# noegroup/bgflow

Hardware: AMD Instinct MI355X
Metric: flow samples/s (fwd+log|detJ|) at batch 2^20 (higher is better)
Workload: dtype f32 (split-f16 conditioner GEMMs: hi+lo f16 operand pairs, f32 accumulate)

## Files before the change

bgflow_amd/_lib.py:

```python
import ctypes
import os

import torch

_HERE = os.path.dirname(os.path.abspath(__file__))
LIB_PATH = os.environ.get("BGK_LIB") or os.path.join(_HERE, "libbgflow_amd.so")
_lib = None

i32, i64, f32, f64, vp = ctypes.c_int32, ctypes.c_int64, ctypes.c_float, ctypes.c_double, ctypes.c_void_p

_SIGNATURES = {
    "bgk_abi_version": (ctypes.c_int, []),
    "bgk_last_error": (ctypes.c_char_p, []),
    "bgk_set_option": (ctypes.c_int, [i32, i32]),
    "bgk_detmath_probe": (ctypes.c_int, [vp, i64, i32, vp, vp]),
    "bgk_rqs_transform": (ctypes.c_int, [vp, i64, vp, i64, i32, vp, i64, i32, i32, i32,
                                         f64, f64, f64, f64, f64, f64, f64, i32,
                                         vp, i64, vp, i32, vp, vp, vp]),
    "bgk_rqs_backward": (ctypes.c_int, [vp, i64, vp, i64, i32, vp, i64, i32, i32, i32,
                                        f64, f64, f64, f64, f64, f64, f64, i32,
                                        vp, i64, vp, vp, i64, vp, i64, vp, i32, vp]),
    "bgk_affine_transform": (ctypes.c_int, [vp, i64, vp, i64, vp, i64, vp, i32, i32, i32, i64, i32,
                                            vp, i64, vp, i32, vp]),
    "bgk_affine_backward": (ctypes.c_int, [vp, i64, vp, i64, vp, i64, vp, i32, i32, i32, i64, i32,
# ... 18 lines not shown
                                     vp, vp, vp, i64, vp, i64, vp, i32, vp, vp]),
    "bgk_ic_ic2xyz": (ctypes.c_int, [vp, vp, vp, i64, vp, i64, vp, i32, vp, i32, i32, f32, i32,
                                     vp, vp, i32, f32, i64, vp, i64, vp, i32, vp, vp]),
    "bgk_ic_refsys": (ctypes.c_int, [vp, i64, i32, i32, f32, i32, vp, vp, i32, vp]),
    "bgk_icdf_ic2xyz": (ctypes.c_int, [vp, vp, vp, i64, vp, i64, vp, vp, vp, vp, i32, f32, vp, i32, vp, i32, i32, f32, i32,
                                       vp, vp, i32, f32, i64, vp, i64, vp, i32, vp, vp]),
    "bgk_icdf_ic2xyz_reg": (ctypes.c_int, [vp, vp, vp, vp, vp, i32, f32, vp, i32, vp, i32, f32, i32, vp, vp, i32, f64, i64,
                                           vp, i64, vp, i32, vp, vp]),
    "bgk_icdf_ic2xyz_uni": (ctypes.c_int, [vp, vp, vp, vp, vp, i32, f32, vp, i32, vp, i32, f32, i32, vp, vp, i32, f64, i64,
                                           vp, i64, vp, i32, vp, vp]),
    "bgk_icdf_ic2xyz_uni_train": (ctypes.c_int, [vp, vp, vp, vp, vp, i32, f32, vp, i32, vp, i32, f32, i32, vp, vp, i32, f64, i64,
                                                 vp, i64, vp, i32, vp, vp, vp, vp, vp, vp]),
    "bgk_icdf_ic2xyz_uni_train_kl": (ctypes.c_int, [vp, vp, vp, vp, vp, i32, f32, vp, i32, vp, i32, f32, i32, vp, vp, i32, f64, i64,
                                                    vp, i64, vp, vp, vp, vp, vp, vp, vp, f64, f64, f64, i32, vp, vp, vp, vp, vp]),
    "bgk_xyz2ic_cdf_uni": (ctypes.c_int, [vp, vp, i32, f32, vp, i32, vp, i32, f32, i32, vp, vp, i32, f64, i64,
                                          vp, vp, vp, vp, vp, i32, vp, vp]),
    "bgk_ic_ic2xyz_backward": (ctypes.c_int, [vp, vp, vp, i64, vp, i64, vp, i32, vp, i32, i32, f32, i32, vp, i32, i64,
                                              vp, i64, vp, vp, vp, vp, i64, vp, i64, vp, vp]),
    "bgk_cdf_transform": (ctypes.c_int, [vp, i64, vp, i64, i32, i32, i32, f32, vp, i64, vp, i32, vp]),
    "bgk_cdf_backward": (ctypes.c_int, [vp, i64, vp, i64, vp, i64, i32, i32, i32, f32, vp, i64, vp, vp, i64, vp]),
    "bgk_ic_xyz2ic_backward": (ctypes.c_int, [vp, i64, vp, i32, vp, i32, i32, f32, i32, vp, i32, i64,
                                              vp, vp, vp, i64, vp, i64, vp, vp, i64, vp]),
    "bgk_ic_refsys_backward": (ctypes.c_int, [vp, vp, vp, i64, i32, i32, f32, i32, vp, vp]),
    "bgk_coupling_rqs_dense": (ctypes.c_int, [vp, i64, i32, i32, vp, vp, vp, i32, i32, i32,
                                              vp, i64, i64, i32, i32, ctypes.c_uint64, i32,
                                              f64, f64, f64, f64, f64, f64, f64, i32,
                                              vp, i64, vp, i32, vp, vp, vp]),
    "bgk_coupling_rqs_dense_h2": (ctypes.c_int, [vp, i64, i32, i32, vp, vp, vp, f32, f32, f32, vp, i32, i32, i32, i32,
                                                 vp, i64, i64, i32, i32, ctypes.c_uint64, i32,
                                                 f64, f64, f64, f64, f64, f64, f64, i32,
                                                 vp, i64, vp, i32, vp, vp, vp]),
    "bgk_coupling_rqs_dense_deep": (ctypes.c_int, [vp, i64, i32, i32, vp, vp, vp, f32, vp, f32, i32, i32,
                                                   vp, i64, i64, i32, i32, ctypes.c_uint64, i32,
                                                   f64, f64, f64, f64, f64, f64, f64, i32,
                                                   vp, i64, vp, i32, vp, vp, vp]),
    "bgk_coupling_rqs_dense_h2_mc": (ctypes.c_int, [vp, vp, vp, i32, i32, vp, vp, vp, f32, f32, f32, vp, i32, i32, i32, i32,
                                                    vp, i64, i64, i32, i32, ctypes.c_uint64, i32,
                                                    f64, f64, f64, f64, f64, f64, f64, i32,
                                                    vp, i64, vp, i32, vp, vp, vp]),
    "bgk_coupling_affine_dense_h2_mc": (ctypes.c_int, [vp, vp, vp, i32, i32,
                                                       vp, vp, vp, f32, f32, f32, i32, vp, vp, vp, f32, f32, f32, i32,
                                                       i32, vp, i32, i32, i32, vp, i64, i64, i32, vp, i64, vp, i32, vp]),
    "bgk_coupling_affine_dense_h3_mc": (ctypes.c_int, [vp, vp, vp, i32, i32,
                                                       vp, vp, vp, vp, f32, f32, f32, f32, i32, vp, vp, vp, vp, f32, f32, f32, f32, i32,
                                                       i32, vp, i32, i32, i32, vp, i64, i64, i32, vp, i64, vp, i32, vp]),
    "bgk_pack_dense_h2": (ctypes.c_int, [vp, vp, i32, i32, vp, vp, vp, vp, i32, vp, i32, i32, i32, vp, vp, vp, vp, vp]),
    "bgk_coupling_rqs_dense_h2_train": (ctypes.c_int, [vp, i64, i32, i32, vp, vp, vp, f32, f32, f32, vp, i32, i32, i32,
                                                       vp, i64, i64, i32, i32, ctypes.c_uint64, i32,
                                                       f64, f64, f64, f64, f64, f64, f64, i32,
                                                       vp, i64, vp, i32, vp, vp, vp, vp, i64, vp, i32, vp]),
    "bgk_coupling_rqs_dense_h2_backward": (ctypes.c_int, [vp, vp, f32, vp, i32, i32, vp, i64, i64, i32, i32, i32, ctypes.c_uint64, i32,
                                                          f64, f64, f64, f64, f64, f64, f64, i32,
                                                          vp, i64, vp, vp, i64, vp, i64, vp, vp]),
    "bgk_coupling_affine_dense_h2": (ctypes.c_int, [vp, i64, i32, i32,
                                                    vp, vp, vp, f32, f32, f32, i32, vp, vp, vp, f32, f32, f32, i32,
                                                    i32, vp, i32, i32, i32, vp, i64, i64, i32, vp, i64, vp, i32, vp]),
    "bgk_coupling_affine_dense_h3": (ctypes.c_int, [vp, i64, i32, i32,
                                                    vp, vp, vp, vp, f32, f32, f32, f32, i32, vp, vp, vp, vp, f32, f32, f32, f32, i32,
                                                    i32, vp, i32, i32, i32, vp, i64, i64, i32, vp, i64, vp, i32, vp]),
    "bgk_coupling_affine_dense_deep": (ctypes.c_int, [vp, i64, i32, i32,
                                                      vp, vp, vp, f32, vp, f32, i32, vp, vp, vp, f32, vp, f32, i32,
                                                      i32, i32, vp, i32, i32, i32, vp, i64, i64, i32, vp, i64, vp, i32, vp]),
    "bgk_pack_dense_h2_t": (ctypes.c_int, [vp, i32, vp, vp, i32, vp, vp, vp, vp, vp]),
    "bgk_dense_backward_dx": (ctypes.c_int, [vp, i64, i32, vp, vp, vp, i64, i32, i32, vp, vp, vp, vp, i32, i64,
                                             vp, vp, vp, vp, vp, i64, vp, i64, vp, vp, vp]),
    "bgk_dense_weight_grad_reduce_many": (ctypes.c_int, [i32] + [vp] * 10 + [i32, vp]),
    "bgk_pack_dense_h2_many": (ctypes.c_int, [i32] + [vp] * 14 + [vp]),
    "bgk_pack_dense_h2_t_many": (ctypes.c_int, [i32] + [vp] * 9 + [vp]),
    "bgk_column_sum": (ctypes.c_int, [vp, i64, i64, i32, vp, i32, vp, vp]),
    "bgk_absmax": (ctypes.c_int, [vp, i64, i64, i32, vp, vp]),
    "bgk_whiten": (ctypes.c_int, [vp, i64, vp, vp, vp, i32, i32, i64, vp, i64, vp]),
    "bgk_normal_energy": (ctypes.c_int, [vp, i64, vp, i32, i64, f64, f64, vp, vp]),
    "bgk_normal_energy_backward": (ctypes.c_int, [vp, i64, vp, i32, i64, f64, vp, vp, i64, vp]),
    "bgk_energy_fields": (ctypes.c_int, [vp, vp, vp, vp, vp, vp, i32, i64, f64, f64, f64, vp, vp, i32, vp, i32, vp, vp]),
    "bgk_energy_fields_backward": (ctypes.c_int, [vp, vp, vp, vp, vp, vp, i32, i64, f64, vp, vp, vp, vp, i32, vp, vp, vp, vp]),
    "bgk_philox_fields": (ctypes.c_int, [ctypes.c_uint64, ctypes.c_uint32, i64, i32, vp, vp, vp, vp, vp, vp, vp, vp, f64, i64, vp, vp]),
    "bgk_colmap": (ctypes.c_int, [vp, i32, vp, i32, vp, vp, ctypes.c_uint64, ctypes.c_uint32, i64, i64, vp, i32, f64, vp, vp]),
    "bgk_grad_nan_flag":(ctypes.c_int, [vp, i64, vp, vp]),
    "bgk_adam_step": (ctypes.c_int, [vp, vp, vp, vp, i64, f32, f32, f32, f32, f32, i64, vp, vp, vp]),
    "bgk_dense_weight_grad_workspace": (i64, [i64, i32, i32]),
    "bgk_dense_weight_grad": (ctypes.c_int, [vp, i64, i32, vp, vp, vp, vp, i32, vp, i64, i32, i32, i64, vp, i64,
                                             vp, vp, vp, vp, vp, vp, i32, vp, vp]),
    "bgk_pack_rqs_columns": (i32, [i32, i32, vp, vp]),
    "bgk_dense_layer": (ctypes.c_int, [vp, i64, i64, i32, vp, i32, f32, vp, vp, i32, i32, vp, i64, i32, vp]),
    "bgk_pack_linear_layer": (ctypes.c_int, [vp, i64, i32, i32, vp, vp, vp]),
    "bgk_dense_layer_steps": (ctypes.c_int, [i32]),
    "bgk_refresh_linear_layer": (ctypes.c_int, [vp, i64, i32, i32, i32, vp, vp, vp, vp]),
    "bgk_activation": (ctypes.c_int, [vp, i64, i64, i32, i32, vp, i64, vp]),
    "bgk_activation_backward": (ctypes.c_int, [vp, i64, vp, i64, i64, i32, i32, vp, i64, vp]),
    "bgk_affine_net_backward64_workspace": (i64, [i64, i32, i32, i32, i32]),
    "bgk_affine_net_backward64": (ctypes.c_int, [vp, i64, i32, vp, vp, vp, i64, i32, i32, i32, vp, vp, vp, vp, i32, i64,
                                                 vp, i64, vp, i64, vp, vp, i64, vp, vp, vp, vp, vp, vp, i32, vp]),
    "bgk_affine_coupling_backward64_workspace": (i64, [i64, i32, i32, i32, i32, i32, i32]),
    "bgk_affine_coupling_backward64": (ctypes.c_int, [vp, i64, i32, vp, i64, i32, vp, i64, vp,
                                                      vp, vp, vp, vp, vp, i64,
                                                      vp, vp, vp, vp, vp, vp, i32, i32, i32,
                                                      vp, vp, vp, vp, vp, vp, vp, i32, i32, i32,
                                                      vp, i32, i64, vp, i64, vp, vp, i64, vp, i64, vp, vp, i64, vp, vp, i32, vp]),
    "bgk_linear_weight_grad_workspace": (i64, [i64, i32, i32]),
    "bgk_linear_weight_grad": (ctypes.c_int, [vp, i64, i32, vp, i64, i32, i64, vp, i64, vp, vp, i32, vp, vp]),
}

ABI_SYMBOLS = tuple(_SIGNATURES)


def lib():
    global _lib
    if _lib is None:
        if not os.path.exists(LIB_PATH):
            raise RuntimeError(
                f"{LIB_PATH} is missing: the MI355X kernels are not built. Run `python -m bgflow_amd.build` "
                "(hipcc, gfx950). bgflow_amd has no CPU fallback.")
        try:
            handle = ctypes.CDLL(LIB_PATH)
        except OSError as e:
            raise RuntimeError(f"cannot load {LIB_PATH}: {e}. bgflow_amd has no CPU fallback.") from e
        for name, (res, args) in _SIGNATURES.items():
            fn = getattr(handle, name)
            fn.restype = res
            fn.argtypes = args
        _lib = handle
    return _lib


def check(status, what):
    if status != 0:
        msg = lib().bgk_last_error().decode(errors="replace")
        if status == -1 and "Minimal bin" in msg:
            raise ValueError(msg)
        raise RuntimeError(f"{what} failed (status {status}): {msg}")


def require_hip(*tensors):
    for t in tensors:
        if t is None:
            continue
        if not t.is_cuda:
            raise RuntimeError(
                "bgflow_amd kernels run on MI355X (HIP) tensors only; got a tensor on "
                f"'{t.device}'. There is no CPU fallback in this package.")
        if t.dtype not in (torch.float32, torch.int32):
            raise RuntimeError(f"bgflow_amd kernels are float32; got {t.dtype}")


def ptr(t):
    return None if t is None else ctypes.c_void_p(t.data_ptr())


def cond_segments(parts):
    rows = [rowmajor(t) for t in parts]
    n = len(rows)
    ptrs = (ctypes.c_void_p * n)(*[t.data_ptr() for t, _ in rows])
    lds = (ctypes.c_int64 * n)(*[ld for _, ld in rows])
    widths = (ctypes.c_int32 * n)(*[t.shape[1] for t, _ in rows])
    return ptrs, lds, widths, n, rows


def stream_ptr(device=None):
    return ctypes.c_void_p(torch.cuda.current_stream(device).cuda_stream)


def rowmajor(t):
    assert t.dim() == 2, "expected [batch, features]"
    if t.stride(1) != 1 and t.shape[1] > 1:
        t = t.contiguous()
    if t.shape[1] == 1 and t.stride(1) != 1:
# ... 7 lines not shown
```

bgflow_amd/csrc/bgk_fused.hip:

```cpp
#include "bgk_mfma_h2.h"
#include "bgk_fused2.h"

namespace {

typedef float f32x16 __attribute__((ext_vector_type(16)));

constexpr int FW = 4;
constexpr int FTHREADS = FW * 64;
constexpr int HID = 128;
constexpr int KB = 8;
constexpr int PPD = 3 * KB + 1;
constexpr int DPC = 128 / PPD;
constexpr int PF = 4;
constexpr int LDS_P = 128 * 32;
constexpr int SROW = 33;

struct FusedArgs {
    const float* cond; int64_t ldc; int d_c; int periodic;
    const float4* W0; int T0;
    const float4* W1;
    const float4* W2; int n_chunks;
    int last_tiles;
    int act;
    const float* y; int64_t ldy;
// ... 1203 lines not shown
extern "C" int32_t bgk_pack_rqs_columns(int32_t d, int32_t K, const int32_t* nc_slot_host, int32_t* src_col) {
    if (d <= 0 || K <= 0 || 3 * K + 1 > 128) return BGK_EINVAL;
    const int ppd = 3 * K + 1, dpc = 128 / ppd;
    const int n_chunks = (d + dpc - 1) / dpc;
    const int ncp = n_chunks * 128;
    if (src_col) {
        for (int i = 0; i < ncp; ++i) src_col[i] = -1;
        for (int jd = 0; jd < d; ++jd) {
            const int c = jd / dpc, q = jd - c * dpc;
            int32_t* dst = src_col + c * 128 + q * ppd;
            for (int k = 0; k < K; ++k) {
                dst[k] = jd * K + k;
                dst[K + k] = d * K + jd * K + k;
                dst[2 * K + k] = 2 * d * K + jd * K + k;
            }
            const int slot = nc_slot_host ? nc_slot_host[jd] : -1;
            dst[3 * K] = slot >= 0 ? 3 * d * K + slot : -1;
        }
    }
    return ncp;
}

extern "C" int bgk_coupling_rqs_dense(const float* cond, int64_t ldc, int32_t d_c, int32_t periodic,
                                      const float* W0p, const float* W1p, const float* W2p,
                                      int32_t H0, int32_t H1, int32_t act, const float* y,
                                      int64_t ldy, int64_t B, int32_t d, int32_t K, uint64_t circ_mask,
                                      int32_t inverse,
                                      double left, double right, double bottom, double top,
                                      double min_bin_width, double min_bin_height,
                                      double min_derivative, int32_t identity_init, float* out,
                                      int64_t ldo, float* dlogp, int32_t accumulate,
                                      int32_t* bin_idx, int32_t* oob_count, void* stream) {
    if (B == 0) return 0;
    BGK_CHECK_ARG(cond && W0p && W1p && W2p && y && out && dlogp, "bgk_coupling_rqs_dense: null pointer");
    BGK_CHECK_ARG(B >= 0 && d > 0 && d_c > 0, "bgk_coupling_rqs_dense: bad sizes");
    if (H0 != HID || H1 != HID || K != KB || d > 64 || act < 1 || act > 3) {
        bgk_set_error("bgk_coupling_rqs_dense: only hidden=(128,128), n_bins=8, d<=64, act in {SiLU,ReLU,Tanh} are fused "
                      "(got H0=%d H1=%d K=%d d=%d act=%d)", H0, H1, K, d, act);
        return BGK_EUNSUPPORTED;
    }
    const int n_in = periodic ? 2 * d_c : d_c;
    if ((n_in + 9) * SROW > LDS_P) {
        bgk_set_error("bgk_coupling_rqs_dense: conditioner input of %d features does not fit the layer-0 tile", n_in);
        return BGK_EUNSUPPORTED;
    }
    BGK_CHECK_ARG(min_bin_width * K <= 1.0 && min_bin_height * K <= 1.0,
                  "Minimal bin width/height too large for the number of bins");
    if (B == 0) return 0;
    FusedArgs a;
    a.cond = cond; a.ldc = ldc; a.d_c = d_c; a.periodic = periodic;
    a.W0 = reinterpret_cast<const float4*>(W0p); a.T0 = ((n_in + 1) / 2 + 3) & ~3;
    a.W1 = reinterpret_cast<const float4*>(W1p);
    a.W2 = reinterpret_cast<const float4*>(W2p); a.n_chunks = (d + DPC - 1) / DPC;
    a.last_tiles = ((d - (a.n_chunks - 1) * DPC) * PPD + 31) / 32;
    a.act = act; a.y = y; a.ldy = ldy; a.B = B; a.d = d; a.inverse = inverse;
    a.circ_mask = circ_mask;
    a.out = out; a.ldo = ldo; a.dlogp = dlogp; a.accumulate = accumulate;
    a.bin_idx = bin_idx; a.oob_count = oob_count;
    a.lds_per_wave = LDS_P + (d + 1) * SROW;
    a.cfg = bgk_make_rqs_cfg(left, right, bottom, top, min_bin_width, min_bin_height, min_derivative, identity_init, K);
    size_t shmem = sizeof(float) * (size_t)FW * a.lds_per_wave;
    int64_t n_wg = ((B + 31) / 32 + FW - 1) / FW;
    BGK_CHECK_ARG(n_wg < (int64_t)0x7fffffff, "bgk_coupling_rqs_dense: batch too large for one launch");
    int grid = (int)n_wg;
    hipStream_t st = (hipStream_t)stream;
#define BGK_LAUNCH(A, I) hipLaunchKernelGGL((coupling_rqs_dense_kernel<A, I>), dim3(grid), dim3(FTHREADS), shmem, st, a)
    if (act == 1) { if (inverse) BGK_LAUNCH(1, 1); else BGK_LAUNCH(1, 0); }
    else if (act == 2) { if (inverse) BGK_LAUNCH(2, 1); else BGK_LAUNCH(2, 0); }
    else { if (inverse) BGK_LAUNCH(3, 1); else BGK_LAUNCH(3, 0); }
#undef BGK_LAUNCH
    return bgk_launch_status("bgk_coupling_rqs_dense");
}

namespace {
int launch_h2(const char* what, const float* cond, int64_t ldc, int32_t d_c, int32_t periodic,
              const void* A0p, const void* A1p, const void* A2p, float c0, float c1, float c2, const float* cs_dev,
              int32_t operand_dtype, int32_t H0, int32_t H1, int32_t act, const float* y, int64_t ldy, int64_t B, int32_t d, int32_t K,
              uint64_t circ_mask, int32_t inverse, double left, double right, double bottom, double top,
              double min_bin_width, double min_bin_height, double min_derivative, int32_t identity_init,
              float* out, int64_t ldo, float* dlogp, int32_t accumulate, int32_t* bin_idx, int32_t* oob_count,
              float* z0, float* z1, float* params, int64_t ldp, const int32_t* src_col, void* stream, const BgkCondSegs* segs = nullptr,
              int params_layout = 0) {
    if (segs && segs->n >= 1) { cond = segs->ptr[0]; ldc = segs->ld[0]; }
    BGK_CHECK_ARG(cond && A0p && A1p && A2p && y && out && dlogp, "%s: null pointer", what);
    BGK_CHECK_ARG(B >= 0 && d > 0 && d_c > 0, "%s: bad sizes", what);
    const bool other_k = (K == 4 || K == 12 || K == 16 || K == 32) && operand_dtype == 0;
    const bool wide = H0 == 32 * W_T && H1 == 32 * W_T;
    if (wide && (operand_dtype != 0 || z0 || z1 || params || (segs && segs->n > 1))) {
        bgk_set_error("%s: hidden width 256 runs fused in split-f16 inference from one conditioning tensor only", what);
        return BGK_EUNSUPPORTED;
    }
    if ((!wide && (H0 != HID || H1 != HID)) || (K != KB && !other_k) || d > 64 || act < 1 || act > 3) {
        bgk_set_error("%s: only hidden=(128,128), n_bins=8 (4 | 12 | 16 | 32: split-f16 form only), d<=64, act in {SiLU,ReLU,Tanh} are fused "
                      "(got H0=%d H1=%d K=%d d=%d act=%d)", what, H0, H1, K, d, act);
        return BGK_EUNSUPPORTED;
    }
    const int n_in = periodic ? 2 * d_c : d_c;
    const int S0 = (n_in + 1 + 15) / 16;
    if (16 * S0 * SROW > LDS_P) {
        bgk_set_error("%s: conditioner input of %d features does not fit the layer-0 tile (at most 111)", what, n_in);
        return BGK_EUNSUPPORTED;
    }
    BGK_CHECK_ARG(min_bin_width * K <= 1.0 && min_bin_height * K <= 1.0,
                  "Minimal bin width/height too large for the number of bins");
    if (B == 0) return 0;
    if (wide) {
        FusedArgsH2 ah;
        FusedArgs& a = ah.f;
        a.cond = cond; a.ldc = ldc; a.d_c = d_c; a.periodic = periodic;
        a.W0 = nullptr; a.W1 = nullptr; a.W2 = nullptr; a.T0 = 0;
        const int ppd_k = 3 * K + 1, dpc_k = 128 / ppd_k;
        a.n_chunks = (d + dpc_k - 1) / dpc_k;
        a.last_tiles = ((d - (a.n_chunks - 1) * dpc_k) * ppd_k + 31) / 32;
        a.act = act; a.y = y; a.ldy = ldy; a.B = B; a.d = d; a.inverse = inverse;
        a.circ_mask = circ_mask;
        a.out = out; a.ldo = ldo; a.dlogp = dlogp; a.accumulate = accumulate;
        a.bin_idx = bin_idx; a.oob_count = oob_count;
        a.lds_per_wave = 128 * 32 + (d + 1) * SROW;
        a.cfg = bgk_make_rqs_cfg(left, right, bottom, top, min_bin_width, min_bin_height, min_derivative, identity_init, K);
        ah.A0 = reinterpret_cast<const uint4*>(A0p); ah.S0 = S0;
        ah.A1 = reinterpret_cast<const uint4*>(A1p);
        ah.A2 = reinterpret_cast<const uint4*>(A2p);
        ah.c0 = c0; ah.c1 = c1; ah.c2 = c2; ah.cs_dev = cs_dev;
        ah.z0 = nullptr; ah.z1 = nullptr; ah.params = nullptr; ah.ldp = 0; ah.src_col = nullptr;
        const size_t shmem = sizeof(float) * (size_t)FW * a.lds_per_wave;
        const int64_t n_wg = ((B + 31) / 32 + FW - 1) / FW;
        BGK_CHECK_ARG(n_wg < (int64_t)0x7fffffff, "%s: batch too large for one launch", what);
        const int grid = (int)n_wg;
        hipStream_t st = (hipStream_t)stream;
#define BGK_LAUNCHW(I, KK) hipLaunchKernelGGL((coupling_rqs_dense_w256_kernel<I, KK>), dim3(grid), dim3(FTHREADS), shmem, st, ah)
#define BGK_LAUNCHW2(KK) do { if (inverse) BGK_LAUNCHW(1, KK); else BGK_LAUNCHW(0, KK); } while (0)
        if (K == 8) BGK_LAUNCHW2(8); else if (K == 4) BGK_LAUNCHW2(4); else if (K == 12) BGK_LAUNCHW2(12);
        else if (K == 16) BGK_LAUNCHW2(16); else BGK_LAUNCHW2(32);
#undef BGK_LAUNCHW2
#undef BGK_LAUNCHW
        return bgk_launch_status(what);
    }
    const bool v2_ok = bgk_h2_variant == 2 && K == KB && ldc < (1 << 24) && ldy < (1 << 24) && ldo < (1 << 24);
    if (segs && segs->n > 1 && !v2_ok) return BGK_EUNSUPPORTED;
    if (params_layout == 1 && !(v2_ok && z0 != nullptr && operand_dtype == 0 && params && z1)) return BGK_EUNSUPPORTED;
    if (params_layout == 2 && !(v2_ok && z0 != nullptr && operand_dtype == 0 && z1)) return BGK_EUNSUPPORTED;
    if (v2_ok && z0 != nullptr && operand_dtype == 0 && (src_col || params_layout >= 1) && (params || params_layout == 2) && z1)
        return bgk_launch_rqs_dense_h2v2_train(what, z0, z1, params_layout == 2 ? nullptr : params, ldp, params_layout >= 1 ? nullptr : src_col, cond, ldc, d_c, periodic, A0p, A1p, A2p, c0, c1, c2, cs_dev,
                                               act, y, ldy, B, d, circ_mask, inverse, left, right, bottom, top, min_bin_width,
                                               min_bin_height, min_derivative, identity_init, out, ldo, dlogp, accumulate, bin_idx,
                                               oob_count, stream, segs);
    if (v2_ok && z0 == nullptr && operand_dtype == 1)
        return bgk_launch_rqs_dense_h2v2_bf16(what, cond, ldc, d_c, periodic, A0p, A1p, A2p, c0, c1, c2, cs_dev, act, y, ldy, B, d, circ_mask,
                                              inverse, left, right, bottom, top, min_bin_width, min_bin_height, min_derivative,
                                              identity_init, out, ldo, dlogp, accumulate, bin_idx, oob_count, stream, segs);
    if (v2_ok && z0 == nullptr && operand_dtype == 0)
        return bgk_launch_rqs_dense_h2v2(what, cond, ldc, d_c, periodic, A0p, A1p, A2p, c0, c1, c2, cs_dev, act, y, ldy, B, d, circ_mask,
                                         inverse, left, right, bottom, top, min_bin_width, min_bin_height, min_derivative,
                                         identity_init, out, ldo, dlogp, accumulate, bin_idx, oob_count, stream, segs);
    FusedArgsH2 ah;
    FusedArgs& a = ah.f;
    a.cond = cond; a.ldc = ldc; a.d_c = d_c; a.periodic = periodic;
    a.W0 = nullptr; a.W1 = nullptr; a.W2 = nullptr; a.T0 = 0;
    const int ppd_k = 3 * K + 1, dpc_k = 128 / ppd_k;
    a.n_chunks = (d + dpc_k - 1) / dpc_k;
    a.last_tiles = ((d - (a.n_chunks - 1) * dpc_k) * ppd_k + 31) / 32;
    a.act = act; a.y = y; a.ldy = ldy; a.B = B; a.d = d; a.inverse = inverse;
    a.circ_mask = circ_mask;
    a.out = out; a.ldo = ldo; a.dlogp = dlogp; a.accumulate = accumulate;
    a.bin_idx = bin_idx; a.oob_count = oob_count;
    const bool save = z0 != nullptr;
    a.lds_per_wave = 128 * (save ? 33 : 32) + (d + 1) * SROW;
    a.cfg = bgk_make_rqs_cfg(left, right, bottom, top, min_bin_width, min_bin_height, min_derivative, identity_init, K);
    ah.A0 = reinterpret_cast<const uint4*>(A0p); ah.S0 = S0;
    ah.A1 = reinterpret_cast<const uint4*>(A1p);
    ah.A2 = reinterpret_cast<const uint4*>(A2p);
    ah.c0 = c0; ah.c1 = c1; ah.c2 = c2; ah.cs_dev = cs_dev;
    ah.z0 = z0; ah.z1 = z1; ah.params = params; ah.ldp = ldp; ah.src_col = src_col;
    size_t shmem = sizeof(float) * (size_t)FW * a.lds_per_wave;
    int64_t n_wg = ((B + 31) / 32 + FW - 1) / FW;
    BGK_CHECK_ARG(n_wg < (int64_t)0x7fffffff, "%s: batch too large for one launch", what);
    int grid = (int)n_wg;
    hipStream_t st = (hipStream_t)stream;
    BGK_CHECK_ARG(operand_dtype == 0 || (operand_dtype == 1 && !save), "%s: operand_dtype %d (0 = split-f16, 1 = bf16; the training "
                  "forward is split-f16 only)", what, operand_dtype);
#define BGK_LAUNCH(A, I, S, F) hipLaunchKernelGGL((coupling_rqs_dense_h2_kernel<A, I, S, F>), dim3(grid), dim3(FTHREADS), shmem, st, ah)
#define BGK_LAUNCH2(A, I) do { if (save) BGK_LAUNCH(A, I, true, false); else if (operand_dtype == 1) BGK_LAUNCH(A, I, false, true); \
                               else BGK_LAUNCH(A, I, false, false); } while (0)
#define BGK_LAUNCHK(A, I, S, KK) hipLaunchKernelGGL((coupling_rqs_dense_h2_kernel<A, I, S, false, KK>), dim3(grid), dim3(FTHREADS), shmem, st, ah)
#define BGK_LAUNCHK3(A, I, KK) do { if (save) BGK_LAUNCHK(A, I, true, KK); else BGK_LAUNCHK(A, I, false, KK); } while (0)
#define BGK_LAUNCHK2(A, I) do { if (K == 4) BGK_LAUNCHK3(A, I, 4); else if (K == 12) BGK_LAUNCHK3(A, I, 12); \
                                else if (K == 16) BGK_LAUNCHK3(A, I, 16); else BGK_LAUNCHK3(A, I, 32); } while (0)
    if (K != KB) {
        if (act == 1) { if (inverse) BGK_LAUNCHK2(1, 1); else BGK_LAUNCHK2(1, 0); }
        else if (act == 2) { if (inverse) BGK_LAUNCHK2(2, 1); else BGK_LAUNCHK2(2, 0); }
        else { if (inverse) BGK_LAUNCHK2(3, 1); else BGK_LAUNCHK2(3, 0); }
    }
    else if (act == 1) { if (inverse) BGK_LAUNCH2(1, 1); else BGK_LAUNCH2(1, 0); }
    else if (act == 2) { if (inverse) BGK_LAUNCH2(2, 1); else BGK_LAUNCH2(2, 0); }
    else { if (inverse) BGK_LAUNCH2(3, 1); else BGK_LAUNCH2(3, 0); }
#undef BGK_LAUNCHK2
#undef BGK_LAUNCHK3
#undef BGK_LAUNCHK
#undef BGK_LAUNCH2
#undef BGK_LAUNCH
    return bgk_launch_status(what);
}
}

extern "C" int bgk_coupling_rqs_dense_deep(const float* cond, int64_t ldc, int32_t d_c, int32_t periodic,
                                           const void* A0p, const void* A1p, const void* A2p, float c0, const float* c1s, float c2,
                                           int32_t n_hidden, int32_t act, const float* y, int64_t ldy, int64_t B, int32_t d, int32_t K,
                                           uint64_t circ_mask, int32_t inverse,
                                           double left, double right, double bottom, double top,
                                           double min_bin_width, double min_bin_height, double min_derivative, int32_t identity_init,
                                           float* out, int64_t ldo, float* dlogp, int32_t accumulate,
                                           int32_t* bin_idx, int32_t* oob_count, void* stream) {
    if (B == 0) return 0;
    const char* what = "bgk_coupling_rqs_dense_deep";
    BGK_CHECK_ARG(cond && A0p && A2p && y && out && dlogp, "%s: null pointer", what);
    BGK_CHECK_ARG(B > 0 && d > 0 && d_c > 0, "%s: bad sizes", what);
    BGK_CHECK_ARG(n_hidden == 1 || (A1p && c1s), "%s: null hidden-layer operands", what);
    if (n_hidden < 1 || n_hidden > DEEP_MAX_HH + 1 || !(K == 4 || K == 8 || K == 12 || K == 16 || K == 32) || d > 64 || act < 1 || act > 3) {
        bgk_set_error("%s: 1 .. %d hidden layers of width 128, n_bins in {4, 8, 12, 16, 32}, d<=64, act in {SiLU,ReLU,Tanh} are fused "
                      "(got n_hidden=%d K=%d d=%d act=%d)", what, DEEP_MAX_HH + 1, n_hidden, K, d, act);
        return BGK_EUNSUPPORTED;
    }
    const int n_in = periodic ? 2 * d_c : d_c;
    const int S0 = (n_in + 1 + 15) / 16;
    if (16 * S0 * SROW > LDS_P) {
        bgk_set_error("%s: conditioner input of %d features does not fit the layer-0 tile (at most 111)", what, n_in);
        return BGK_EUNSUPPORTED;
    }
    BGK_CHECK_ARG(min_bin_width * K <= 1.0 && min_bin_height * K <= 1.0, "Minimal bin width/height too large for the number of bins");
    DeepArgs da;
    FusedArgsH2& ah = da.h;
    FusedArgs& a = ah.f;
    a.cond = cond; a.ldc = ldc; a.d_c = d_c; a.periodic = periodic;
    a.W0 = nullptr; a.W1 = nullptr; a.W2 = nullptr; a.T0 = 0;
    const int ppd_k = 3 * K + 1, dpc_k = 128 / ppd_k;
    a.n_chunks = (d + dpc_k - 1) / dpc_k;
    a.last_tiles = ((d - (a.n_chunks - 1) * dpc_k) * ppd_k + 31) / 32;
// ... 115 lines not shown
```

bgflow_amd/csrc/bgk_fused2.h:

```cpp
#ifndef BGK_FUSED2_H
#define BGK_FUSED2_H
#include <stdint.h>

#define BGK_MAX_COND 3
struct BgkCondSegs { const float* ptr[BGK_MAX_COND]; int64_t ld[BGK_MAX_COND]; int32_t w[BGK_MAX_COND]; int32_t n; };

int bgk_launch_rqs_dense_h2v2(const char* what, const float* cond, int64_t ldc, int32_t d_c, int32_t periodic,
                              const void* A0p, const void* A1p, const void* A2p, float c0, float c1, float c2, const float* cs_dev,
                              int32_t act, const float* y, int64_t ldy, int64_t B, int32_t d, uint64_t circ_mask, int32_t inverse,
                              double left, double right, double bottom, double top,
                              double min_bin_width, double min_bin_height, double min_derivative, int32_t identity_init,
                              float* out, int64_t ldo, float* dlogp, int32_t accumulate, int32_t* bin_idx, int32_t* oob_count,
                              void* stream, const BgkCondSegs* segs = nullptr);

int bgk_launch_rqs_dense_h2v2_train(const char* what, float* z0, float* z1, float* params, int64_t ldp, const int32_t* src_col,
                                    const float* cond, int64_t ldc, int32_t d_c, int32_t periodic,
                                    const void* A0p, const void* A1p, const void* A2p, float c0, float c1, float c2, const float* cs_dev,
                                    int32_t act, const float* y, int64_t ldy, int64_t B, int32_t d, uint64_t circ_mask, int32_t inverse,
                                    double left, double right, double bottom, double top,
                                    double min_bin_width, double min_bin_height, double min_derivative, int32_t identity_init,
                                    float* out, int64_t ldo, float* dlogp, int32_t accumulate, int32_t* bin_idx, int32_t* oob_count,
                                    void* stream, const BgkCondSegs* segs = nullptr);

int bgk_launch_rqs_bwd_recompute(const char* what, const float* z1, const void* A2p, float c2, const float* cs_dev, int32_t act,
                                 const float* y, int64_t ldy, int64_t B, int32_t d, uint64_t circ_mask, int32_t inverse,
                                 double left, double right, double bottom, double top,
                                 double min_bin_width, double min_bin_height, double min_derivative, int32_t identity_init,
                                 const float* g_out, int64_t ldgo, const float* g_dlogp, float* g_y, int64_t ldgy,
                                 float* g_params, int64_t ldgp, float* g_absmax, void* stream);

int bgk_launch_rqs_dense_h2v2_bf16(const char* what, const float* cond, int64_t ldc, int32_t d_c, int32_t periodic,
                                   const void* A0p, const void* A1p, const void* A2p, float c0, float c1, float c2, const float* cs_dev,
                                   int32_t act, const float* y, int64_t ldy, int64_t B, int32_t d, uint64_t circ_mask, int32_t inverse,
                                   double left, double right, double bottom, double top,
                                   double min_bin_width, double min_bin_height, double min_derivative, int32_t identity_init,
                                   float* out, int64_t ldo, float* dlogp, int32_t accumulate, int32_t* bin_idx, int32_t* oob_count,
                                   void* stream, const BgkCondSegs* segs = nullptr);

int bgk_launch_affine_dense_v2(const float* cond, int64_t ldc, int32_t d_c, int32_t periodic,
                               const void* sA0, const void* sA1, const void* sA1b, const void* sA2, float sc0, float sc1, float sc1b, float sc2, int32_t s_act,
                               const void* tA0, const void* tA1, const void* tA1b, const void* tA2, float tc0, float tc1, float tc1b, float tc2, int32_t t_act,
                               const float* log_alpha, int32_t preserve_volume, int32_t is_circular, int32_t inverse,
                               const float* y, int64_t ldy, int64_t B, int32_t d,
                               float* out, int64_t ldo, float* dlogp, int32_t accumulate, void* stream, const BgkCondSegs* segs = nullptr);

struct BgkAffTrainSave { const float* s_cs; float* s_z0; float* s_z1; const float* t_cs; float* t_z0; float* t_z1; float* mu; float* s_raw; int64_t ldms;
                         int64_t ldz; };
int bgk_launch_affine_dense_v2_train(const BgkAffTrainSave* save, const float* cond, int64_t ldc, int32_t d_c, int32_t periodic,
                               const void* sA0, const void* sA1, const void* sA1b, const void* sA2, float sc0, float sc1, float sc1b, float sc2, int32_t s_act,
                               const void* tA0, const void* tA1, const void* tA1b, const void* tA2, float tc0, float tc1, float tc1b, float tc2, int32_t t_act,
                               const float* log_alpha, int32_t preserve_volume, int32_t is_circular, int32_t inverse,
                               const float* y, int64_t ldy, int64_t B, int32_t d,
                               float* out, int64_t ldo, float* dlogp, int32_t accumulate, void* stream, const BgkCondSegs* segs = nullptr);

extern int bgk_h2_variant;
extern int bgk_rc_vjp_variant;

#endif
```

bgflow_amd/csrc/bgk_fused2.hip:

```cpp
#include "bgk_common.h"
#include "bgk_fused2.h"

#ifndef BGK_V2_SAVE
#define BGK_V2_SAVE 0
#endif
#if BGK_V2_SAVE
#include "bgk_mfma_h2.h"
#include "bgk_rqs_vjp.h"
#define coupling_rqs_dense_h2v2_kernel coupling_rqs_dense_h2v2_train_kernel
#endif
#ifndef BGK_V2_BF16
#define BGK_V2_BF16 0
#endif
#if BGK_V2_BF16
#define coupling_rqs_dense_h2v2_kernel coupling_rqs_dense_h2v2_bf16_kernel
typedef short s16x8 __attribute__((ext_vector_type(8)));
#endif
#ifndef BGK_V2_AFFTRAIN
#define BGK_V2_AFFTRAIN 0
#endif
#if BGK_V2_AFFTRAIN
#define coupling_affine_dense_v2_kernel coupling_affine_dense_v2_train_kernel
#endif
constexpr int NPROD = BGK_V2_BF16 ? 1 : 3;

namespace {

typedef float f32x16 __attribute__((ext_vector_type(16)));
typedef _Float16 h16x8 __attribute__((ext_vector_type(8)));
typedef unsigned u32x4 __attribute__((ext_vector_type(4)));

constexpr int FW = 4;
constexpr int FTHREADS = FW * 64;
constexpr int KB = 8;
constexpr int PPD = 3 * KB + 1;
constexpr int DPC = 128 / PPD;
constexpr int SROW = 33;
constexpr int ST = BGK_V2_SAVE ? 33 : 32;
constexpr int KS = 8;
constexpr int GBLK = KS * 8 + 4;
#ifndef BGK_V2_KARG
#define BGK_V2_KARG 2
#endif
#ifndef BGK_V2_RD
#define BGK_V2_RD 4
#endif
#ifndef BGK_V2_TS
#define BGK_V2_TS 0
#endif
#if BGK_V2_TS
#define V2_TS(k) do { const unsigned long long t_ = __builtin_amdgcn_s_memtime(); if (lane == 0 && a.bin_idx) a.bin_idx[b0 * d + (k)] = (int)(unsigned)t_; } while (0)
#else
#define V2_TS(k) do { } while (0)
#endif
constexpr int RD = BGK_V2_RD;
constexpr int EH = 34;

struct CondSegs {
    const float* ptr[BGK_MAX_COND]; int64_t ld[BGK_MAX_COND]; int w[BGK_MAX_COND]; int off[BGK_MAX_COND]; uint32_t magic[BGK_MAX_COND];
    int n;
};

struct SetK { float gnum, low, high, dstep; float kc[7]; };

struct SpC {
    float left, right;
    SetK sa, sb;
    float beta, kout, min_d;
};

struct V2Args {
    CondSegs cs;
    int d_c; int periodic;
    const float* y; int64_t ldy; float* out; int64_t ldo; int d; uint32_t magic_d;
    int64_t B; float* dlogp; int accumulate; int32_t* bin_idx; int32_t* oob_count;
    const uint4* A0; const uint4* A1; const uint4* A2; int S0; int n_chunks; int last_tiles;
    float c0, c1, c2; const float* cs_dev;
    uint64_t circ_mask;
    SpC sc;
    int lds_per_wave;
    int nfs, ys, stage, y_dma, out_lin;
#if BGK_V2_SAVE
    float* z0; float* z1;
    float* params; int64_t ldp;
    const int32_t* src_col;
#endif
};
typedef const __attribute__((address_space(4))) V2Args* kargs_t;

struct BFrag { h16x8 hi[KS], lo[KS]; };
struct TFrag { u32x4 hi, lo; };

__device__ __forceinline__ int drow(int m, int r, int hh) { return 32 * m + (r & 3) + 8 * (r >> 2) + 4 * hh; }

template <int NT, int MS = 4, int RDX = RD>
struct Live {
    static constexpr int NTS = KS * NT;
    static constexpr int NEV = NPROD * NTS + NT;
    f32x16 (&out)[4];
    const BFrag& b;
    const uint4* W;
    unsigned voff;
    TFrag (&ring)[RDX];
    __amdgpu_buffer_rsrc_t rs;

    template <int BLK>
    __device__ __forceinline__ u32x4 blk() {
        return __builtin_amdgcn_raw_buffer_load_b128(rs, voff + ((BLK * 1024) & 4095), (BLK * 1024) & ~4095, 0);
    }
    template <int T>
    __device__ __forceinline__ void load() {
        if constexpr (T < NTS) {
            constexpr int s = T / NT, m = T % NT;
#if BGK_V2_BF16
            ring[T % RDX].hi = blk<(s * MS + m) * 2>();
#else
            ring[T % RDX].hi = blk<(s * MS + m) * 2>();
            ring[T % RDX].lo = blk<(s * MS + m) * 2 + 1>();
#endif
        } else if constexpr (T < NTS + NT) {
            ring[T % RDX].hi = blk<KS * MS * 2 + (T - NTS)>();
        }
    }
    template <int T0, int T1>
    __device__ __forceinline__ void loads() {
        if constexpr (T0 < T1) { load<T0>(); loads<T0 + 1, T1>(); }
    }
    __device__ __forceinline__ void start() {
        __builtin_amdgcn_sched_barrier(0);
        rs = __builtin_amdgcn_make_buffer_rsrc((void*)W, 0, 0x7fffffff, 0x00020000);
        loads<0, RDX>();
        __builtin_amdgcn_sched_barrier(0);
    }
    template <int E>
    __device__ __forceinline__ void event() {
        __builtin_amdgcn_sched_barrier(0);
#if BGK_V2_BF16
        if constexpr (E < NTS) {
            constexpr int T = E, s = T / NT, m = T % NT;
            const s16x8 a = __builtin_bit_cast(s16x8, ring[T % RDX].hi), bb = __builtin_bit_cast(s16x8, b.hi[s]);
            if constexpr (s == 0) {
                const f32x16 z = {0.f, 0.f, 0.f, 0.f, 0.f, 0.f, 0.f, 0.f, 0.f, 0.f, 0.f, 0.f, 0.f, 0.f, 0.f, 0.f};
                out[m] = __builtin_amdgcn_mfma_f32_32x32x16_bf16(a, bb, z, 0, 0, 0);
            } else {
                out[m] = __builtin_amdgcn_mfma_f32_32x32x16_bf16(a, bb, out[m], 0, 0, 0);
            }
            load<T + RDX>();
        } else if constexpr (E < NEV) {
            constexpr int m = E - NTS, T = NTS + m;
            const s16x8 one2 = {(short)0x3f80, (short)0x3f80, 0, 0, 0, 0, 0, 0};
            out[m] = __builtin_amdgcn_mfma_f32_32x32x16_bf16(__builtin_bit_cast(s16x8, ring[T % RDX].hi), one2, out[m], 0, 0, 0);
        }
#else
        if constexpr (E < 3 * NTS) {
            constexpr int T = E / 3, p = E % 3, s = T / NT, m = T % NT;
            const TFrag& f = ring[T % RDX];
            const h16x8 a = __builtin_bit_cast(h16x8, p == 0 ? f.lo : f.hi);
            const h16x8 bb = p == 1 ? b.lo[s] : b.hi[s];
            if constexpr (s == 0 && p == 0) {
                const f32x16 z = {0.f, 0.f, 0.f, 0.f, 0.f, 0.f, 0.f, 0.f, 0.f, 0.f, 0.f, 0.f, 0.f, 0.f, 0.f, 0.f};
                out[m] = __builtin_amdgcn_mfma_f32_32x32x16_f16(a, bb, z, 0, 0, 0);
            } else {
                out[m] = __builtin_amdgcn_mfma_f32_32x32x16_f16(a, bb, out[m], 0, 0, 0);
            }
            if constexpr (p == 2) load<T + RDX>();
        } else if constexpr (E < NEV) {
            constexpr int m = E - 3 * NTS, T = NTS + m;
            const h16x8 one2 = {(_Float16)1.0f, (_Float16)1.0f, 0, 0, 0, 0, 0, 0};
            out[m] = __builtin_amdgcn_mfma_f32_32x32x16_f16(__builtin_bit_cast(h16x8, ring[T % RDX].hi), one2, out[m], 0, 0, 0);
        }
#endif
        __builtin_amdgcn_sched_barrier(0);
    }
    template <int E0, int E1>
    __device__ __forceinline__ void events() {
        if constexpr (E0 < E1) {
            event<E0>();
            events<E0 + 1, E1>();
        }
    }
    template <int HK, int NH>
    __device__ __forceinline__ void hook() {
        constexpr int e0 = (HK * NEV) / NH, e1 = ((HK + 1) * NEV) / NH;
        if constexpr (e0 < e1) events<e0, e1>();
    }
};
struct NoLive {
    template <int HK, int NH> __device__ __forceinline__ void hook() {}
};

template <class G, int BASE, int NH>
struct Hooks {
    G& g;
    template <int I> __device__ __forceinline__ void at() { g.template hook<BASE + I, NH>(); }
};

template <int ACT, int T, int P, class H>
__device__ __forceinline__ void act_split_pair(H& hk, const f32x16& t, float c, BFrag& bf) {
    constexpr int r = 2 * P;
    float a0, a1;
    if constexpr (ACT == 2) {
        a0 = t[r] * c; a1 = t[r + 1] * c;
        hk.template at<3 * P>();
        a0 = a0 > 0.0f ? a0 : 0.0f; a1 = a1 > 0.0f ? a1 : 0.0f;
        hk.template at<3 * P + 1>();
    } else {
        constexpr float kk = ACT == 1 ? -1.44269504088896341f : 2.88539008177792681f;
        const float ck = c * kk, rc = 1.0f / c;
        const float e0 = __builtin_amdgcn_exp2f(t[r] * ck), e1 = __builtin_amdgcn_exp2f(t[r + 1] * ck);
        hk.template at<3 * P>();
        if constexpr (ACT == 1) {
            const float q0 = __builtin_amdgcn_rcpf(__builtin_fmaf(e0, rc, rc)), q1 = __builtin_amdgcn_rcpf(__builtin_fmaf(e1, rc, rc));
            a0 = t[r] * q0; a1 = t[r + 1] * q1;
        } else {
            const float q0 = __builtin_amdgcn_rcpf(1.0f + e0), q1 = __builtin_amdgcn_rcpf(1.0f + e1);
            a0 = 1.0f - 2.0f * q0; a1 = 1.0f - 2.0f * q1;
        }
        hk.template at<3 * P + 1>();
    }
    constexpr int s = 2 * T + (r >> 3), e = r & 7;
#if BGK_V2_BF16
    typedef __bf16 bf2v __attribute__((ext_vector_type(2)));
    typedef float f2v __attribute__((ext_vector_type(2)));
    typedef _Float16 h2v __attribute__((ext_vector_type(2)));
    const bf2v pb = __builtin_convertvector((f2v){a0, a1}, bf2v);
    const h2v ph = __builtin_bit_cast(h2v, pb);
    bf.hi[s][e] = ph[0]; bf.hi[s][e + 1] = ph[1];
#else
    unsigned uh, ul;
    asm("v_cvt_pk_f16_f32 %0, %1, %2" : "=v"(uh) : "v"(a0), "v"(a1));
    asm("v_fma_mixlo_f16 %0, %1, -1.0, %2 op_sel:[0,0,0] op_sel_hi:[1,0,0]" : "=v"(ul) : "v"(uh), "v"(a0));
    asm("v_fma_mixhi_f16 %0, %1, -1.0, %2 op_sel:[1,0,0] op_sel_hi:[1,0,0]" : "+v"(ul) : "v"(uh), "v"(a1));
    typedef _Float16 h2v __attribute__((ext_vector_type(2)));
    const h2v ph = __builtin_bit_cast(h2v, uh), pl = __builtin_bit_cast(h2v, ul);
    bf.hi[s][e] = ph[0]; bf.hi[s][e + 1] = ph[1];
    bf.lo[s][e] = pl[0]; bf.lo[s][e + 1] = pl[1];
#endif
    hk.template at<3 * P + 2>();
}
template <int ACT, int T, class H>
__device__ __forceinline__ void act_split_tile(H hk, const f32x16& t, float c, BFrag& bf) {
    act_split_pair<ACT, T, 0>(hk, t, c, bf); act_split_pair<ACT, T, 1>(hk, t, c, bf);
    act_split_pair<ACT, T, 2>(hk, t, c, bf); act_split_pair<ACT, T, 3>(hk, t, c, bf);
    act_split_pair<ACT, T, 4>(hk, t, c, bf); act_split_pair<ACT, T, 5>(hk, t, c, bf);
    act_split_pair<ACT, T, 6>(hk, t, c, bf); act_split_pair<ACT, T, 7>(hk, t, c, bf);
}

struct SpK { float kL, kz, c2; };

__device__ __forceinline__ float fdiv_hw(float n, float d) {
    const float r = __builtin_amdgcn_rcpf(d);
    const float q = n * r;
    return __builtin_fmaf(__builtin_fmaf(-d, q, n), r, q);
}
__device__ __forceinline__ float rcp_nr(float d) {
    const float r = __builtin_amdgcn_rcpf(d);
    return __builtin_fmaf(__builtin_fmaf(-d, r, 1.0f), r, r);
}

template <bool KARG> struct ScSrc;
template <> struct ScSrc<true> {
    kargs_t ka;
    __device__ __forceinline__ ScSrc(const V2Args&) { ka = (kargs_t)__builtin_amdgcn_kernarg_segment_ptr(); asm volatile("" : "+s"(ka)); }
    __device__ __forceinline__ const __attribute__((address_space(4))) SpC& get() const { return ka->sc; }
};
template <> struct ScSrc<false> {
    const V2Args& a;
    __device__ __forceinline__ ScSrc(const V2Args& a_) : a(a_) {}
    __device__ __forceinline__ const SpC& get() const { return a.sc; }
};

template <int INV, class H>
__device__ __forceinline__ float rqs_fast(H hk, float x, const float* pa, const float* pb, const float* ps, bool circ,
                                          const V2Args& a, const SpK& k, float* lad, int* bin, int* oob) {
    const ScSrc<(BGK_V2_KARG == 2 ? INV != 0 : BGK_V2_KARG != 0)> scs(a);
#define SC scs.get()
    float va[KB], vb[KB];
#pragma unroll
    for (int i = 0; i < KB; ++i) va[i] = pa[i * ST];
#pragma unroll
    for (int i = 0; i < KB; ++i) vb[i] = pb[i * ST];
    *oob = (x < SC.left) | (x > SC.right);
    x = __builtin_amdgcn_fmed3f(x, SC.left, SC.right);
    float mA = __builtin_fmaxf(__builtin_fmaxf(va[0], va[1]), va[2]);
    mA = __builtin_fmaxf(__builtin_fmaxf(mA, va[3]), va[4]);
    mA = __builtin_fmaxf(__builtin_fmaxf(mA, va[5]), va[6]);
    mA = __builtin_fmaxf(mA, va[7]);
    const float nmA = -(mA * k.kL);
    hk.template at<0>();
    float E[KB];
    E[0] = __builtin_amdgcn_exp2f(__builtin_fmaf(va[0], k.kL, nmA));
    E[1] = __builtin_amdgcn_exp2f(__builtin_fmaf(va[1], k.kL, nmA));
    E[2] = __builtin_amdgcn_exp2f(__builtin_fmaf(va[2], k.kL, nmA));
    hk.template at<1>();
    E[3] = __builtin_amdgcn_exp2f(__builtin_fmaf(va[3], k.kL, nmA));
    E[4] = __builtin_amdgcn_exp2f(__builtin_fmaf(va[4], k.kL, nmA));
    E[5] = __builtin_amdgcn_exp2f(__builtin_fmaf(va[5], k.kL, nmA));
    hk.template at<2>();
    E[6] = __builtin_amdgcn_exp2f(__builtin_fmaf(va[6], k.kL, nmA));
    E[7] = __builtin_amdgcn_exp2f(__builtin_fmaf(va[7], k.kL, nmA));
    E[1] += E[0]; E[2] += E[1];
    hk.template at<3>();
    E[3] += E[2]; E[4] += E[3]; E[5] += E[4]; E[6] += E[5]; E[7] += E[6];
    hk.template at<4>();
    const float gA = SC.sa.gnum * rcp_nr(E[7]);
    float kn[7];
    kn[0] = __builtin_fmaf(E[0], gA, SC.sa.kc[0]);
    kn[1] = __builtin_fmaf(E[1], gA, SC.sa.kc[1]);
    hk.template at<5>();
    kn[2] = __builtin_fmaf(E[2], gA, SC.sa.kc[2]);
    kn[3] = __builtin_fmaf(E[3], gA, SC.sa.kc[3]);
    kn[4] = __builtin_fmaf(E[4], gA, SC.sa.kc[4]);
    kn[5] = __builtin_fmaf(E[5], gA, SC.sa.kc[5]);
    kn[6] = __builtin_fmaf(E[6], gA, SC.sa.kc[6]);
    hk.template at<6>();
    float low_a = SC.sa.low, high_a = SC.sa.high;
    asm volatile("" : "+s"(low_a), "+s"(high_a));
#pragma unroll
    for (int i = 0; i < 7; ++i) asm volatile("" : "+v"(kn[i]));
    const bool g3 = x >= kn[3];
    hk.template at<7>();
    float w0 = g3 ? kn[3] : low_a, w1 = g3 ? kn[4] : kn[0], w2 = g3 ? kn[5] : kn[1], w3 = g3 ? kn[6] : kn[2];
    hk.template at<8>();
    float w4 = g3 ? high_a : kn[3];
    const bool gm = x >= w2;
    const float v0 = gm ? w2 : w0, v1 = gm ? w3 : w1, v2 = gm ? w4 : w2;
    hk.template at<9>();
    const bool gl = x >= v1;
    const float lo = gl ? v1 : v0, hi = gl ? v2 : v1;
    float idxf = g3 ? 4.0f : 0.0f;
    hk.template at<10>();
    idxf += gm ? 2.0f : 0.0f;
    idxf += gl ? 1.0f : 0.0f;
    const int idx = (int)idxf;
    *bin = idx;
    hk.template at<11>();
    const int j1 = circ ? ((idx + 1) & 7) : (idx + 1);
    const float s_lo = ps[idx * ST], s_hi = ps[j1 * ST];
    const float A_i = hi - lo;
    float mB = __builtin_fmaxf(__builtin_fmaxf(vb[0], vb[1]), vb[2]);
    hk.template at<12>();
    mB = __builtin_fmaxf(__builtin_fmaxf(mB, vb[3]), vb[4]);
    mB = __builtin_fmaxf(__builtin_fmaxf(mB, vb[5]), vb[6]);
    mB = __builtin_fmaxf(mB, vb[7]);
    const float nmB = -(mB * k.kL);
    float F[KB];
    F[0] = __builtin_amdgcn_exp2f(__builtin_fmaf(vb[0], k.kL, nmB));
    hk.template at<13>();
    F[1] = __builtin_amdgcn_exp2f(__builtin_fmaf(vb[1], k.kL, nmB));
    F[2] = __builtin_amdgcn_exp2f(__builtin_fmaf(vb[2], k.kL, nmB));
    F[3] = __builtin_amdgcn_exp2f(__builtin_fmaf(vb[3], k.kL, nmB));
    hk.template at<14>();
    F[4] = __builtin_amdgcn_exp2f(__builtin_fmaf(vb[4], k.kL, nmB));
    F[5] = __builtin_amdgcn_exp2f(__builtin_fmaf(vb[5], k.kL, nmB));
    F[6] = __builtin_amdgcn_exp2f(__builtin_fmaf(vb[6], k.kL, nmB));
    hk.template at<15>();
    F[7] = __builtin_amdgcn_exp2f(__builtin_fmaf(vb[7], k.kL, nmB));
    F[1] += F[0]; F[2] += F[1]; F[3] += F[2];
    hk.template at<16>();
    F[4] += F[3]; F[5] += F[4]; F[6] += F[5]; F[7] += F[6];
    const float rB = __builtin_amdgcn_rcpf(F[7]);
    hk.template at<17>();
    const float gB = SC.sb.gnum * __builtin_fmaf(__builtin_fmaf(-F[7], rB, 1.0f), rB, rB);
    const float f0 = g3 ? F[3] : 0.0f, f1 = g3 ? F[4] : F[0], f2 = g3 ? F[5] : F[1];
    hk.template at<18>();
    const float f3 = g3 ? F[6] : F[2], f4 = g3 ? F[7] : F[3];
    const float u0 = gm ? f2 : f0, u1 = gm ? f3 : f1, u2 = gm ? f4 : f2;
    hk.template at<19>();
    const float Flo = gl ? u1 : u0;
    float Fhi = gl ? u2 : u1;
    hk.template at<20>();
    const float cb = __builtin_fmaf(idxf, SC.sb.dstep, SC.sb.low);
    hk.template at<21>();
    const float b_i = __builtin_fmaf(Flo, gB, cb);
    float b_ip1 = __builtin_fmaf(Fhi, gB, cb + SC.sb.dstep);
    float top_b = SC.sb.high;
    asm volatile("" : "+s"(top_b));
    b_ip1 = (g3 && gm && gl) ? top_b : b_ip1;
    const float B_i = b_ip1 - b_i;
    const float z0 = s_lo * k.kz;
    hk.template at<22>();
    const float ez0 = __builtin_amdgcn_exp2f(z0);
    float lg0 = __builtin_amdgcn_logf(1.0f + ez0);
    asm volatile("" : "+v"(lg0));
    const float sm0 = ez0 * __builtin_fmaf(ez0, -0.5f, 1.0f) * 1.44269504088896341f;
    hk.template at<23>();
    float l0 = (ez0 < 2.44140625e-4f ? sm0 : lg0) * SC.kout;
    asm volatile("" : "+v"(l0));
    l0 = z0 > 28.8539008177792681f ? s_lo * k.c2 : l0;
    const float d_i = SC.min_d + l0;
    const float z1 = s_hi * k.kz;
    hk.template at<24>();
    const float ez1 = __builtin_amdgcn_exp2f(z1);
    float lg1 = __builtin_amdgcn_logf(1.0f + ez1);
    asm volatile("" : "+v"(lg1));
    const float sm1 = ez1 * __builtin_fmaf(ez1, -0.5f, 1.0f) * 1.44269504088896341f;
    hk.template at<25>();
    float l1 = (ez1 < 2.44140625e-4f ? sm1 : lg1) * SC.kout;
    asm volatile("" : "+v"(l1));
    l1 = z1 > 28.8539008177792681f ? s_hi * k.c2 : l1;
    const float d_ip1 = SC.min_d + l1;
    float cw_i, W_i, ch_i, H_i;
    if (INV) { cw_i = lo; W_i = A_i; ch_i = b_i; H_i = B_i; }
    else { ch_i = lo; H_i = A_i; cw_i = b_i; W_i = B_i; }
    hk.template at<26>();
    const float delta = fdiv_hw(H_i, W_i);
    const float S = d_i + d_ip1 - 2.0f * delta;
    hk.template at<27>();
    float outv, l;
    if (!INV) {
        const float dx = x - ch_i;
        const float dxS = dx * S;
        const float qa = dxS + H_i * (delta - d_i);
        const float qb = H_i * d_i - dxS;
        hk.template at<28>();
        const float qc = -delta * dx;
        const float disc = qb * qb - 4.0f * qa * qc;
        const float sq = __builtin_amdgcn_sqrtf(disc);
        hk.template at<29>();
        const float root = fdiv_hw(2.0f * qc, -qb - sq);
        outv = __builtin_fmaf(root, W_i, cw_i);
        hk.template at<30>();
        const float omr = 1.0f - root;
        const float t1mt = root * omr;
        const float den = delta + S * t1mt;
        const float lden = __builtin_amdgcn_logf(den);
        hk.template at<31>();
        const float num = (delta * delta) * (d_ip1 * (root * root) + 2.0f * delta * t1mt + d_i * (omr * omr));
        hk.template at<32>();
        l = (2.0f * lden - __builtin_amdgcn_logf(num)) * 0.693147180559945309f;
    } else {
        const float theta = fdiv_hw(x - cw_i, W_i);
        const float omt = 1.0f - theta;
        hk.template at<28>();
        const float t1mt = theta * omt;
        const float numer = H_i * (delta * (theta * theta) + d_i * t1mt);
        const float den = delta + S * t1mt;
        hk.template at<29>();
        outv = ch_i + fdiv_hw(numer, den);
        const float lden = __builtin_amdgcn_logf(den);
        hk.template at<30>();
        const float inner = d_ip1 * (theta * theta) + 2.0f * delta * t1mt;
        hk.template at<31>();
        const float num = (delta * delta) * (inner + d_i * (omt * omt));
        hk.template at<32>();
        l = (__builtin_amdgcn_logf(num) - 2.0f * lden) * 0.693147180559945309f;
    }
    hk.template at<33>();
    *lad = l;
    return outv;
}

#undef SC

template <int INV, int IT, int NHK, class G>
__device__ __forceinline__ void spline_slot(G& g, const V2Args& a, const SpK& k, const float* s_p, float* s_y, int c, int nd,
                                            int hh, int j, int rows, float& run, int& oob_local, int (&bins)[3]) {
    const int q = 2 * IT + hh;
    const bool valid = q < nd;
    const int qq = valid ? q : 0;
    const int dim = c * DPC + qq;
    const float* pw = s_p + (qq * PPD) * ST + j;
    const float* ph = pw + KB * ST;
    const float* ps = ph + KB * ST;
    const bool circ = (a.circ_mask >> dim) & 1ull;
    int bin, oob;
    float lad;
    const float x = s_y[j * a.ys + dim];
    Hooks<G, IT * EH, NHK> hk{g};
    const float o = rqs_fast<INV>(hk, x, INV ? pw : ph, INV ? ph : pw, ps, circ, a, k, &lad, &bin, &oob);
    s_y[valid ? j * a.ys + dim : 32 * a.ys + j] = o;
    oob_local += (valid && j < rows) ? oob : 0;
    bins[IT] = bin;
    lad = valid ? lad : 0.0f;
    float l0 = lad, l1 = lad;
    asm volatile("s_nop 1\n\tv_permlane32_swap_b32 %0, %1" : "+v"(l0), "+v"(l1));
    run += l0;
    run += l1;
}

__device__ __forceinline__ void chunk_to_lds(const f32x16 (&h)[4], float* s_p, int hh, int j) {
#pragma unroll
    for (int m = 0; m < 4; ++m)
#pragma unroll
        for (int r = 0; r < 16; ++r) s_p[drow(m, r, hh) * ST + j] = h[m][r];
    __builtin_amdgcn_fence(__ATOMIC_ACQ_REL, "wavefront");
    __builtin_amdgcn_wave_barrier();
}

#if BGK_V2_SAVE
__device__ __forceinline__ void save_chunk_params(const V2Args& a, const float* s_p, int c, int lane, int64_t b0, int rows) {
    if (a.params == nullptr) return;
    if (a.src_col == nullptr) {
        typedef float f4s __attribute__((ext_vector_type(4), aligned(4)));
        const int l = lane & 31, half = lane >> 5;
        const int nd = (a.d - c * DPC) < DPC ? (a.d - c * DPC) : DPC;
        const bool mine = 4 * l < nd * PPD;
        for (int jj = 0; jj < rows; jj += 2) {
            const int r = jj + half;
            if (r < rows && mine) {
                float* prow = a.params + (b0 + r) * a.ldp + (DPC * PPD) * c;
                const f4s v = {s_p[(4 * l) * ST + r] * a.c2, s_p[(4 * l + 1) * ST + r] * a.c2, s_p[(4 * l + 2) * ST + r] * a.c2, s_p[(4 * l + 3) * ST + r] * a.c2};
                *reinterpret_cast<f4s*>(prow + 4 * l) = v;
            }
        }
        return;
    }
    const int col_lo = a.src_col[c * 128 + lane], col_hi = a.src_col[c * 128 + 64 + lane];
    for (int jj = 0; jj < rows; ++jj) {
        float* prow = a.params + (b0 + jj) * a.ldp;
        if (col_lo >= 0) prow[col_lo] = s_p[lane * ST + jj] * a.c2;
        if (col_hi >= 0) prow[col_hi] = s_p[(64 + lane) * ST + jj] * a.c2;
    }
}
#endif

template <int INV, int NT, bool SAVEP>
__device__ __forceinline__ void chunk_piped(const V2Args& a, const SpK& k, float* s_p, float* s_y, int c, int hh, int j, int rows,
                                            float& run, int& oob_local, int (&bins)[3], f32x16 (&h)[4], const BFrag& bf,
                                            TFrag (&ring)[RD], unsigned voff, int64_t b0) {
    Live<NT> g{h, bf, a.A2 + (size_t)(c + 1) * GBLK * 64, voff, ring};
    g.start();
    chunk_to_lds(h, s_p, hh, j);
#if BGK_V2_SAVE
    if constexpr (SAVEP) save_chunk_params(a, s_p, c, (int)threadIdx.x & 63, b0, rows);
#endif
    __builtin_amdgcn_sched_barrier(0);
    spline_slot<INV, 0, 3 * EH>(g, a, k, s_p, s_y, c, DPC, hh, j, rows, run, oob_local, bins);
    spline_slot<INV, 1, 3 * EH>(g, a, k, s_p, s_y, c, DPC, hh, j, rows, run, oob_local, bins);
    spline_slot<INV, 2, 3 * EH>(g, a, k, s_p, s_y, c, DPC, hh, j, rows, run, oob_local, bins);
}

typedef const __attribute__((address_space(1))) void* gvp_t;
typedef __attribute__((address_space(3))) void* lvp_t;
__device__ __forceinline__ void dma_tile32(float* dst, const float* __restrict__ src, int n, int valid, int lane) {
    for (int c = 0; c < n; c += 256) {
        const int e = c + lane * 4;
        if (e + 3 < valid) __builtin_amdgcn_global_load_lds((gvp_t)(src + e), (lvp_t)(dst + c), 16, 0, 0);
    }
    if (valid & 3) {
        const int edge = valid & ~3;
        if (lane < (valid & 3)) __builtin_amdgcn_global_load_lds((gvp_t)(src + edge + lane), (lvp_t)(dst + edge), 4, 0, 0);
    }
}

__device__ __forceinline__ void v2_sincos2pi(float x, float* s, float* c) {
    const float f = __builtin_amdgcn_fractf(x);
    *s = __builtin_amdgcn_sinf(f);
    *c = __builtin_amdgcn_cosf(f);
}

struct StageTiles { int d_c, periodic, nfs, ys, stage, y_dma, d; uint32_t magic_d; int rows, lane; };

__device__ __forceinline__ void stage_issue(const StageTiles& t, const CondSegs& cs, int64_t b0, const float* y_t, float* s_p, float* s_y) {
    if (t.y_dma) dma_tile32(s_y, y_t, 32 * t.d, t.rows * t.d, t.lane);
    if (t.stage == 1) dma_tile32(s_p, cs.ptr[0] + b0 * cs.ld[0], 32 * t.d_c, t.rows * t.d_c, t.lane);
    else if (t.stage == 2) dma_tile32(s_p + 32 * t.nfs, cs.ptr[0] + b0 * cs.ld[0], 32 * t.d_c, t.rows * t.d_c, t.lane);
}

#ifndef BGK_V2_SB
#define BGK_V2_SB 8
#endif
template <class KA>
__device__ __forceinline__ void stage_finish(const StageTiles& t, const CondSegs& cs, int64_t b0, const float* y_t, int ldy32,
                                             float* s_p, float* s_y, float y_fill) {
    constexpr int SB = BGK_V2_SB;
    const int lane = t.lane, rows = t.rows, d = t.d, nfs = t.nfs, n_y = 32 * t.d;
    if (!t.y_dma) {
        for (int base = 0; base < n_y; base += 64 * SB) {
            float vy[SB];
#pragma unroll
            for (int u = 0; u < SB; ++u) {
                const int i = base + u * 64 + lane;
                const int r = (int)(__umul24((unsigned)i, t.magic_d) >> 20), c = i - (int)__umul24((unsigned)r, (unsigned)d);
                vy[u] = (i < n_y && r < rows) ? y_t[(int)__umul24((unsigned)r, (unsigned)ldy32) + c] : y_fill;
            }
#pragma unroll
            for (int u = 0; u < SB; ++u) {
                const int i = base + u * 64 + lane;
                const int r = (int)(__umul24((unsigned)i, t.magic_d) >> 20), c = i - (int)__umul24((unsigned)r, (unsigned)d);
                if (i < n_y) s_y[(int)__umul24((unsigned)r, (unsigned)t.ys) + c] = vy[u];
            }
        }
    }
    if (t.stage == 0) {
        typedef const __attribute__((address_space(4))) KA* ka_t;
        const ka_t kseg = (ka_t)__builtin_amdgcn_kernarg_segment_ptr();
        for (int sg = 0; sg < cs.n; ++sg) {
            const float* cond_t = kseg->cs.ptr[sg] + b0 * kseg->cs.ld[sg];
            const int ldc32 = (int)kseg->cs.ld[sg], w_c = kseg->cs.w[sg], n_c = 32 * w_c, col0 = kseg->cs.off[sg];
            const uint32_t magic_c = kseg->cs.magic[sg];
            for (int base = 0; base < n_c; base += 64 * SB) {
                float vc[SB];
#pragma unroll
                for (int u = 0; u < SB; ++u) {
                    const int i = base + u * 64 + lane;
                    const int r = (int)(__umul24((unsigned)i, magic_c) >> 20), c = i - (int)__umul24((unsigned)r, (unsigned)w_c);
                    vc[u] = (i < n_c && r < rows) ? cond_t[(int)__umul24((unsigned)r, (unsigned)ldc32) + c] : 0.0f;
                }
#pragma unroll
                for (int u = 0; u < SB; ++u) {
                    const int i = base + u * 64 + lane;
                    const int r = (int)(__umul24((unsigned)i, magic_c) >> 20), c = i - (int)__umul24((unsigned)r, (unsigned)w_c);
                    if (i < n_c) {
                        float* f = s_p + (int)__umul24((unsigned)r, (unsigned)nfs) + col0 + c;
                        if (t.periodic) {
                            float sv, cv;
                            v2_sincos2pi(vc[u], &sv, &cv);
                            f[0] = cv;
                            f[t.d_c] = sv;
                        } else {
                            f[0] = vc[u];
                        }
                    }
                }
            }
        }
    }
    asm volatile("s_waitcnt vmcnt(0)" ::: "memory");
    __builtin_amdgcn_fence(__ATOMIC_ACQ_REL, "wavefront");
    __builtin_amdgcn_wave_barrier();
    if (t.stage == 2) {
        const float* raw = s_p + 32 * nfs;
        const uint32_t magic_c = cs.magic[0];
        for (int i = lane; i < 32 * t.d_c; i += 64) {
            const int r = (int)(__umul24((unsigned)i, magic_c) >> 20), c = i - (int)__umul24((unsigned)r, (unsigned)t.d_c);
            float sv, cv;
            v2_sincos2pi(raw[i], &sv, &cv);
            float* f = s_p + (int)__umul24((unsigned)r, (unsigned)nfs) + c;
            f[0] = cv;
            f[t.d_c] = sv;
        }
    }
    if (t.stage != 1) {
        __builtin_amdgcn_fence(__ATOMIC_ACQ_REL, "wavefront");
        __builtin_amdgcn_wave_barrier();
    }
}

__device__ __forceinline__ void store_tile32(float* out_t, int ldo32, const float* s_y, int ys, int d, uint32_t magic_d, int rows, int lane, int lin) {
    const int n = rows * d;
    if (lin) {
        for (int i = lane * 4; i + 3 < n; i += 256) *reinterpret_cast<float4*>(out_t + i) = *reinterpret_cast<const float4*>(s_y + i);
        if (lane < (n & 3)) out_t[(n & ~3) + lane] = s_y[(n & ~3) + lane];
    } else {
        for (int i = lane; i < n; i += 64) {
            const int r = (int)(__umul24((unsigned)i, magic_d) >> 20), cc = i - (int)__umul24((unsigned)r, (unsigned)d);
            out_t[(int)__umul24((unsigned)r, (unsigned)ldo32) + cc] = s_y[(int)__umul24((unsigned)r, (unsigned)ys) + cc];
        }
    }
}

struct L0Frag { uint4 v[4][2]; };
__device__ __forceinline__ void l0_request(L0Frag& f, const uint4* A0, int s, int lane) {
#pragma unroll
    for (int m = 0; m < 4; ++m) {
        f.v[m][0] = A0[((s * 4 + m) * 2 + 0) * 64 + lane];
#if !BGK_V2_BF16
        f.v[m][1] = A0[((s * 4 + m) * 2 + 1) * 64 + lane];
#endif
    }
}
__device__ __forceinline__ void l0_step(f32x16 (&h)[4], const L0Frag& fr, const float* f, bool last, int rel0) {
    float v[8];
#pragma unroll
    for (int e = 0; e < 8; ++e) v[e] = f[e];
    if (last) {
#pragma unroll
        for (int e = 0; e < 8; ++e) v[e] = rel0 + e == 0 ? 1.0f : (rel0 + e > 0 ? 0.0f : v[e]);
    }
#if BGK_V2_BF16
    s16x8 bb;
#pragma unroll
    for (int e = 0; e < 8; ++e) bb[e] = __builtin_bit_cast(short, (__bf16)v[e]);
#pragma unroll
    for (int m = 0; m < 4; ++m)
        h[m] = __builtin_amdgcn_mfma_f32_32x32x16_bf16(__builtin_bit_cast(s16x8, fr.v[m][0]), bb, h[m], 0, 0, 0);
#else
    h16x8 bhi, blo;
#pragma unroll
    for (int e = 0; e < 8; ++e) {
        const float c = v[e];
        const _Float16 hv = (_Float16)c;
        bhi[e] = hv;
        blo[e] = (_Float16)(c - (float)hv);
    }
#pragma unroll
    for (int m = 0; m < 4; ++m) h[m] = __builtin_amdgcn_mfma_f32_32x32x16_f16(__builtin_bit_cast(h16x8, fr.v[m][1]), bhi, h[m], 0, 0, 0);
#pragma unroll
    for (int m = 0; m < 4; ++m) h[m] = __builtin_amdgcn_mfma_f32_32x32x16_f16(__builtin_bit_cast(h16x8, fr.v[m][0]), blo, h[m], 0, 0, 0);
#pragma unroll
    for (int m = 0; m < 4; ++m) h[m] = __builtin_amdgcn_mfma_f32_32x32x16_f16(__builtin_bit_cast(h16x8, fr.v[m][0]), bhi, h[m], 0, 0, 0);
#endif
}

template <int ACT, int INV, bool SAVEP = true>
__global__ __launch_bounds__(FTHREADS, 2) void coupling_rqs_dense_h2v2_kernel(V2Args a) {
    if (a.cs_dev) { a.c0 = a.cs_dev[1]; a.c1 = a.cs_dev[3]; a.c2 = a.cs_dev[5]; }
    asm volatile("s_setreg_imm32_b32 hwreg(HW_REG_MODE, 23, 1), 1");
    extern __shared__ __attribute__((aligned(16))) float smem[];
    const int wave = threadIdx.x >> 6;
    float* s_p = smem + (size_t)wave * a.lds_per_wave;
    float* s_y = s_p + 128 * ST;
    const int d = a.d;
    const int64_t n_tiles = (a.B + 31) / 32;
    const int64_t tile = (int64_t)blockIdx.x * FW + wave;
    if (tile >= n_tiles) return;
    const SpK k{a.c2 * 1.44269504088896341f, a.c2 * a.sc.beta * 1.44269504088896341f, a.c2};
    const int n_in = a.periodic ? 2 * a.d_c : a.d_c;
    const int ldy32 = (int)a.ldy, ldo32 = (int)a.ldo;
    const int n_y = 32 * d;

  {
    const int lane = (int)threadIdx.x & 63, j = lane & 31, hh = lane >> 5;
    const unsigned voff = (unsigned)lane * 16u;
    const int64_t b0 = tile * 32;
    const int rows = (int)((a.B - b0) < 32 ? (a.B - b0) : 32);
    const float* y_t = a.y + b0 * a.ldy;
    float* out_t = a.out + b0 * a.ldo;
    V2_TS(0);

    const int nfs = a.nfs, ys = a.ys;
    const StageTiles stg{a.d_c, a.periodic, nfs, ys, a.stage, a.y_dma, d, a.magic_d, rows, lane};
    stage_issue(stg, a.cs, b0, y_t, s_p, s_y);
    f32x16 h[4], acc[4];
    TFrag ring[RD];
    BFrag bf;
    L0Frag fa, fb;
    l0_request(fa, a.A0, 0, lane);
    Live<4> g1{acc, bf, a.A1, voff, ring};
    g1.start();
    V2_TS(12);
    stage_finish<V2Args>(stg, a.cs, b0, y_t, ldy32, s_p, s_y, 0.5f);
    V2_TS(1);

#pragma unroll
    for (int m = 0; m < 4; ++m)
#pragma unroll
        for (int r = 0; r < 16; ++r) h[m][r] = 0.0f;
    {
        const float* frow = s_p + j * nfs + 8 * hh;
        const int rel0 = 16 * (a.S0 - 1) + 8 * hh - n_in;
        for (int s = 0; s < a.S0; s += 2) {
            if (s + 1 < a.S0) l0_request(fb, a.A0, s + 1, lane);
            l0_step(h, fa, frow + 16 * s, s + 1 == a.S0, rel0);
            if (s + 1 < a.S0) {
                if (s + 2 < a.S0) l0_request(fa, a.A0, s + 2, lane);
                l0_step(h, fb, frow + 16 * (s + 1), s + 2 == a.S0, rel0);
            }
        }
    }

    V2_TS(2);
    {
        Live<4>& g = g1;
#if BGK_V2_SAVE
#pragma unroll
        for (int m = 0; m < 4; ++m)
#pragma unroll
            for (int r = 0; r < 16; ++r) h[m][r] *= a.c0;
        h2_store_rows128(h, a.z0, s_p, b0, rows, lane);
        const float c0_act = 1.0f;
#else
        const float c0_act = a.c0;
#endif
        NoLive none;
        act_split_tile<ACT, 0>(Hooks<NoLive, 0, 1>{none}, h[0], c0_act, bf);
        __builtin_amdgcn_sched_barrier(0);
        V2_TS(14);
        act_split_tile<ACT, 1>(Hooks<Live<4>, 0, 100>{g}, h[1], c0_act, bf);
        act_split_tile<ACT, 2>(Hooks<Live<4>, 24, 100>{g}, h[2], c0_act, bf);
        act_split_tile<ACT, 3>(Hooks<Live<4>, 48, 100>{g}, h[3], c0_act, bf);
        __builtin_amdgcn_sched_barrier(0);
        V2_TS(15);
        g.template events<(72 * Live<4>::NEV) / 100, Live<4>::NEV>();
    }

    V2_TS(3);
    float run = 0.0f;
    int oob_local = 0;
    {
        Live<4> g{h, bf, a.A2, voff, ring};
        g.start();
#if BGK_V2_SAVE
#pragma unroll
        for (int m = 0; m < 4; ++m)
#pragma unroll
            for (int r = 0; r < 16; ++r) acc[m][r] *= a.c1;
        h2_store_rows128(acc, a.z1, s_p, b0, rows, lane);
        const float c1_act = 1.0f;
#else
        const float c1_act = a.c1;
#endif
        NoLive none;
        act_split_tile<ACT, 0>(Hooks<NoLive, 0, 1>{none}, acc[0], c1_act, bf);
        __builtin_amdgcn_sched_barrier(0);
        act_split_tile<ACT, 1>(Hooks<Live<4>, 0, 100>{g}, acc[1], c1_act, bf);
        act_split_tile<ACT, 2>(Hooks<Live<4>, 24, 100>{g}, acc[2], c1_act, bf);
        act_split_tile<ACT, 3>(Hooks<Live<4>, 48, 100>{g}, acc[3], c1_act, bf);
        __builtin_amdgcn_sched_barrier(0);
        g.template events<(72 * Live<4>::NEV) / 100, Live<4>::NEV>();
    }
    V2_TS(4);
    for (int c = 0; c < a.n_chunks; ++c) {
        int bins[3] = {0, 0, 0};
        const int nd = (d - c * DPC) < DPC ? (d - c * DPC) : DPC;
        if (c + 2 < a.n_chunks || (c + 2 == a.n_chunks && a.last_tiles > 2)) {
            chunk_piped<INV, 4, SAVEP>(a, k, s_p, s_y, c, hh, j, rows, run, oob_local, bins, h, bf, ring, voff, b0);
        } else if (c + 2 == a.n_chunks) {
            chunk_piped<INV, 2, SAVEP>(a, k, s_p, s_y, c, hh, j, rows, run, oob_local, bins, h, bf, ring, voff, b0);
        } else {
            NoLive none;
            chunk_to_lds(h, s_p, hh, j);
#if BGK_V2_SAVE
            if constexpr (SAVEP) save_chunk_params(a, s_p, c, lane, b0, rows);
#endif
            spline_slot<INV, 0, 1>(none, a, k, s_p, s_y, c, nd, hh, j, rows, run, oob_local, bins);
            if (nd > 2) spline_slot<INV, 1, 1>(none, a, k, s_p, s_y, c, nd, hh, j, rows, run, oob_local, bins);
            if (nd > 4) spline_slot<INV, 2, 1>(none, a, k, s_p, s_y, c, nd, hh, j, rows, run, oob_local, bins);
        }
#if BGK_V2_TS
        V2_TS(5 + c);
#else
        if (a.bin_idx) {
#pragma unroll
            for (int it = 0; it < 3; ++it) {
                const int q = 2 * it + hh;
                if (q < nd && j < rows) a.bin_idx[(b0 + j) * d + c * DPC + q] = bins[it];
            }
        }
#endif
        __builtin_amdgcn_fence(__ATOMIC_ACQ_REL, "wavefront");
        __builtin_amdgcn_wave_barrier();
    }
    if (hh == 0 && j < rows) {
        if (a.accumulate) a.dlogp[b0 + j] += run; else a.dlogp[b0 + j] = run;
    }
    store_tile32(out_t, ldo32, s_y, ys, d, a.magic_d, rows, lane, a.out_lin);
    if (a.oob_count && __builtin_amdgcn_ballot_w64(oob_local != 0)) {
        for (int off = 32; off > 0; off >>= 1) oob_local += __shfl_xor(oob_local, off);
        if (lane == 0) atomicAdd(a.oob_count, oob_local);
    }
    V2_TS(5 + a.n_chunks);
  }
}

struct TilePlan { int nfs, ys, stage, y_dma, out_lin; };
TilePlan plan_tiles(const CondSegs& cs, int d_c, int periodic, const float* y, int64_t ldy, const float* out, int64_t ldo, int d, int tile_floats) {
    const int n_in = periodic ? 2 * d_c : d_c;
    const auto dma_ok = [](const float* p, int64_t ld, int w) { return ld == w && ((uintptr_t)p & 15) == 0 && (w & 7) != 0; };
    TilePlan t;
    t.y_dma = dma_ok(y, ldy, d) ? 1 : 0;
    t.ys = t.y_dma ? d : (d | 1);
    t.out_lin = (t.y_dma && ldo == d && ((uintptr_t)out & 15) == 0) ? 1 : 0;
    const bool c_dma = cs.n == 1 && dma_ok(cs.ptr[0], cs.ld[0], d_c);
    t.stage = (c_dma && !periodic) ? 1 : ((c_dma && periodic && 32 * ((n_in | 1) + d_c) <= tile_floats) ? 2 : 0);
    t.nfs = t.stage == 1 ? d_c : (n_in | 1);
    return t;
}

SetK make_set(double low, double high, double min_bin, int K) {
    SetK s;
    const double span = high - low, scale = 1.0 - min_bin * K;
    s.gnum = (float)((double)(float)span * (double)(float)scale);
    s.low = (float)low; s.high = (float)high;
    s.dstep = (float)((double)(float)span * (double)(float)min_bin);
    for (int k = 0; k < 7; ++k) s.kc[k] = (float)((double)(float)low + (double)(float)span * (double)(float)min_bin * (k + 1));
    return s;
}

uint32_t magic_div(int d) { return (uint32_t)(((1u << 20) + (uint32_t)d - 1) / (uint32_t)d); }

bool make_cond_segs(CondSegs& cs, const float* cond, int64_t ldc, int d_c, const BgkCondSegs* segs) {
    for (int i = 0; i < BGK_MAX_COND; ++i) { cs.ptr[i] = nullptr; cs.ld[i] = 0; cs.w[i] = 0; cs.off[i] = 0; cs.magic[i] = 0; }
    if (!segs || segs->n <= 1) {
        const float* p = segs && segs->n == 1 ? segs->ptr[0] : cond;
        const int64_t ld = segs && segs->n == 1 ? segs->ld[0] : ldc;
        if (!p || d_c <= 0 || ld >= (1 << 24)) return false;
        cs.n = 1; cs.ptr[0] = p; cs.ld[0] = ld; cs.w[0] = d_c; cs.magic[0] = magic_div(d_c);
        return true;
    }
    if (segs->n > BGK_MAX_COND) return false;
    int off = 0;
    for (int i = 0; i < segs->n; ++i) {
        if (!segs->ptr[i] || segs->w[i] <= 0 || segs->ld[i] < segs->w[i] || segs->ld[i] >= (1 << 24)) return false;
        cs.ptr[i] = segs->ptr[i]; cs.ld[i] = segs->ld[i]; cs.w[i] = segs->w[i]; cs.off[i] = off; cs.magic[i] = magic_div(segs->w[i]);
        off += segs->w[i];
    }
    cs.n = segs->n;
    return off == d_c;
}


#if !BGK_V2_SAVE && !BGK_V2_BF16
struct AffV2Net { const uint4* A0; const uint4* A1; const uint4* A1b; const uint4* A2; float c0, c1, c1b, c2;
#if BGK_V2_AFFTRAIN
                  const float* cs;
                  float* z0; float* z1;
#endif
};
struct AffV2Args {
    CondSegs cs; int d_c; int periodic; int S0;
    AffV2Net shift, scale; int has_shift, has_scale;
    const float* log_alpha; int preserve_volume, is_circular, inverse;
    const float* y; int64_t ldy; int64_t B; int d;
    float* out; int64_t ldo; float* dlogp; int accumulate;
    uint32_t magic_d;
    int lds_tile, lds_per_wave;
    int nfs, ys, stage, y_dma, out_lin;
#if BGK_V2_AFFTRAIN
    float* mu_out; float* s_out; int64_t ldms;
    int slab;
    int zt;
#endif
};

#if BGK_V2_AFFTRAIN
template <int NT>
__device__ __forceinline__ void aff_store_tiles(const f32x16 (&t)[4], float* dst, int pitch, float* slab, int64_t b0, int rows, int lane) {
    const int j = lane & 31, hh = lane >> 5;
    const __amdgpu_buffer_rsrc_t rs = __builtin_amdgcn_make_buffer_rsrc((void*)(dst + b0 * pitch), 0, rows * pitch * 4, 0x00020000);
#pragma unroll
    for (int m = 0; m < NT; ++m)
#pragma unroll
// ... 454 lines not shown
    float gmax = 0.0f;
    const RcTile tl{__builtin_amdgcn_make_buffer_rsrc((void*)(a.y + b0 * a.ldy), 0, (int)(rows * a.ldy * 4), 0x00020000),
                    __builtin_amdgcn_make_buffer_rsrc((void*)(a.g_out + b0 * a.ldgo), 0, (int)(rows * a.ldgo * 4), 0x00020000),
                    __builtin_amdgcn_make_buffer_rsrc((void*)(a.g_y + b0 * a.ldgy), 0, (int)(rows * a.ldgy * 4), 0x00020000),
                    __builtin_amdgcn_make_buffer_rsrc((void*)(a.g_params + b0 * a.ldgp), 0, (int)(rows * a.ldgp * 4), 0x00020000),
                    jr * (int)a.ldy * 4, jr * (int)a.ldgo * 4, j * (int)a.ldgy * 4};
    RcIn in = rc_request(tl, 0, 0, a.d < DPC ? a.d : DPC, hh);
    for (int c = 0; c + 1 < a.n_chunks; ++c) {
        if (c + 2 < a.n_chunks || a.last_tiles > 2) rc_chunk<4, 3, FAST>(a, tl, s_p, c, DPC, lane, rows, gl, gmax, in, h, bf, ring, voff, ts);
        else rc_chunk<2, 3, FAST>(a, tl, s_p, c, DPC, lane, rows, gl, gmax, in, h, bf, ring, voff, ts);
    }
    {
        const int c = a.n_chunks - 1, nd = a.d - c * DPC;
        if (nd > 4) rc_chunk<0, 3, FAST>(a, tl, s_p, c, nd, lane, rows, gl, gmax, in, h, bf, ring, voff, ts);
        else if (nd > 2) rc_chunk<0, 2, FAST>(a, tl, s_p, c, nd, lane, rows, gl, gmax, in, h, bf, ring, voff, ts);
        else rc_chunk<0, 1, FAST>(a, tl, s_p, c, nd, lane, rows, gl, gmax, in, h, bf, ring, voff, ts);
    }
    bgk_publish_absmax(a.g_absmax, gmax);
#if BGK_RC_TS
    asm volatile("s_waitcnt vmcnt(0)" ::: "memory");
    unsigned q4;
    RC_Q(q4);
    if (lane == 0) {
        unsigned* o = reinterpret_cast<unsigned*>(a.g_y + b0 * a.ldgy);
        o[0] = q1 - q0; o[1] = q2 - q1; o[2] = q3 - q2; o[3] = ts.lds; o[4] = ts.vjp; o[5] = ts.gemm; o[6] = ts.st; o[7] = q4 - q0;
    }
#endif
}
#endif

}

#if !BGK_V2_SAVE && !BGK_V2_BF16 && !BGK_V2_AFFTRAIN
int bgk_h2_variant = 2;
#endif

#if BGK_V2_SAVE
int bgk_rc_vjp_variant = 2;
int bgk_launch_rqs_bwd_recompute(const char* what, const float* z1, const void* A2p, float c2, const float* cs_dev, int32_t act,
                                 const float* y, int64_t ldy, int64_t B, int32_t d, uint64_t circ_mask, int32_t inverse,
                                 double left, double right, double bottom, double top,
                                 double min_bin_width, double min_bin_height, double min_derivative, int32_t identity_init,
                                 const float* g_out, int64_t ldgo, const float* g_dlogp, float* g_y, int64_t ldgy,
                                 float* g_params, int64_t ldgp, float* g_absmax, void* stream) {
    RcArgs a;
    a.z1 = z1; a.A2 = reinterpret_cast<const uint4*>(A2p); a.c2 = c2; a.cs_dev = cs_dev;
    a.n_chunks = (d + DPC - 1) / DPC;
    a.last_tiles = ((d - (a.n_chunks - 1) * DPC) * PPD + 31) / 32;
    a.y = y; a.ldy = ldy; a.B = B; a.d = d; a.nc_mask = ~circ_mask & (d >= 64 ? ~0ull : ((1ull << d) - 1ull)); a.inverse = inverse;
    BGK_CHECK_ARG(ldy < (1 << 24) && ldgo < (1 << 24) && ldgy < (1 << 24) && ldgp < (1 << 24), "%s: row stride too large", what);
    a.g_out = g_out; a.ldgo = ldgo; a.g_dlogp = g_dlogp; a.g_y = g_y; a.ldgy = ldgy; a.g_params = g_params; a.ldgp = ldgp;
    a.g_absmax = g_absmax;
    a.cfg = bgk_make_rqs_cfg(left, right, bottom, top, min_bin_width, min_bin_height, min_derivative, identity_init, KB);
    a.lds_per_wave = ((128 * ST + 3) / 4) * 4;
    static_assert(128 * ST >= 32 * 128, "the chunk buffer holds the z1 tile");
    const size_t shmem = sizeof(float) * (size_t)FW * a.lds_per_wave;
    const int64_t n_wg = ((B + 31) / 32 + FW - 1) / FW;
    BGK_CHECK_ARG(n_wg < (int64_t)0x7fffffff, "%s: batch too large for one launch", what);
    hipStream_t st = (hipStream_t)stream;
#define BGK_LAUNCH(A, F) do { (void)hipFuncSetAttribute(reinterpret_cast<const void*>(coupling_rqs_bwd_recompute_kernel<A, F>), hipFuncAttributeMaxDynamicSharedMemorySize, 160 * 1024); \
                              hipLaunchKernelGGL((coupling_rqs_bwd_recompute_kernel<A, F>), dim3((int)n_wg), dim3(FTHREADS), shmem, st, a); } while (0)
#define BGK_LAUNCH_F(A) do { if (bgk_rc_vjp_variant == 1) BGK_LAUNCH(A, false); else BGK_LAUNCH(A, true); } while (0)
    if (act == 1) BGK_LAUNCH_F(1); else if (act == 2) BGK_LAUNCH_F(2); else BGK_LAUNCH_F(3);
#undef BGK_LAUNCH_F
#undef BGK_LAUNCH
    return bgk_launch_status(what);
}
#endif

#if !BGK_V2_AFFTRAIN
#if BGK_V2_SAVE
int bgk_launch_rqs_dense_h2v2_train(const char* what, float* z0, float* z1, float* params, int64_t ldp, const int32_t* src_col,
                                    const float* cond, int64_t ldc, int32_t d_c, int32_t periodic,
#elif BGK_V2_BF16
int bgk_launch_rqs_dense_h2v2_bf16(const char* what, const float* cond, int64_t ldc, int32_t d_c, int32_t periodic,
#else
int bgk_launch_rqs_dense_h2v2(const char* what, const float* cond, int64_t ldc, int32_t d_c, int32_t periodic,
#endif
                              const void* A0p, const void* A1p, const void* A2p, float c0, float c1, float c2, const float* cs_dev,
                              int32_t act, const float* y, int64_t ldy, int64_t B, int32_t d, uint64_t circ_mask, int32_t inverse,
                              double left, double right, double bottom, double top,
                              double min_bin_width, double min_bin_height, double min_derivative, int32_t identity_init,
                              float* out, int64_t ldo, float* dlogp, int32_t accumulate, int32_t* bin_idx, int32_t* oob_count,
                              void* stream, const BgkCondSegs* segs) {
    V2Args a;
    const int n_in = periodic ? 2 * d_c : d_c;
    BGK_CHECK_ARG(make_cond_segs(a.cs, cond, ldc, d_c, segs), "%s: bad conditioning segments", what);
    a.d_c = d_c; a.periodic = periodic;
    a.y = y; a.ldy = ldy; a.out = out; a.ldo = ldo; a.d = d; a.magic_d = magic_div(d);
    a.B = B; a.dlogp = dlogp; a.accumulate = accumulate; a.bin_idx = bin_idx; a.oob_count = oob_count;
    a.A0 = reinterpret_cast<const uint4*>(A0p); a.A1 = reinterpret_cast<const uint4*>(A1p); a.A2 = reinterpret_cast<const uint4*>(A2p);
    a.S0 = (n_in + 1 + 15) / 16;
    a.n_chunks = (d + DPC - 1) / DPC;
    a.last_tiles = ((d - (a.n_chunks - 1) * DPC) * PPD + 31) / 32;
    a.c0 = c0; a.c1 = c1; a.c2 = c2; a.cs_dev = cs_dev;
    a.circ_mask = circ_mask;
    a.sc.left = (float)left; a.sc.right = (float)right;
    const SetK sw = make_set(left, right, min_bin_width, KB), sh = make_set(bottom, top, min_bin_height, KB);
    a.sc.sa = inverse ? sw : sh;
    a.sc.sb = inverse ? sh : sw;
    const double beta = identity_init ? (0.6931471805599453 / (1.0 - min_derivative)) : 1.0;
    a.sc.beta = (float)beta; a.sc.kout = (float)(0.6931471805599453 / (double)(float)beta); a.sc.min_d = (float)min_derivative;
    const TilePlan tp = plan_tiles(a.cs, d_c, periodic, y, ldy, out, ldo, d, 128 * ST);
    a.nfs = tp.nfs; a.ys = tp.ys; a.stage = tp.stage; a.y_dma = tp.y_dma; a.out_lin = tp.out_lin;
    BGK_CHECK_ARG(32 * a.nfs + 16 <= 128 * ST, "%s: %d conditioner input features do not fit the LDS tile", what, n_in);
    a.lds_per_wave = ((128 * ST + 32 * a.ys + 32 + 3) / 4) * 4;
#if BGK_V2_SAVE
    a.z0 = z0; a.z1 = z1; a.params = params; a.ldp = ldp; a.src_col = src_col;
#endif
    const size_t shmem = sizeof(float) * (size_t)FW * a.lds_per_wave;
    const int64_t n_wg = ((B + 31) / 32 + FW - 1) / FW;
    BGK_CHECK_ARG(n_wg < (int64_t)0x7fffffff, "%s: batch too large for one launch", what);
    BGK_CHECK_ARG((int64_t)32 * (d > d_c ? d : d_c) < (1 << 16), "%s: tile index range", what);
    BGK_CHECK_ARG(ldy < (1 << 24) && ldo < (1 << 24), "%s: row stride too large", what);
    const int grid = (int)n_wg;
    hipStream_t st = (hipStream_t)stream;
#if BGK_V2_SAVE
#define BGK_LAUNCH(A, I) do { if (params) hipLaunchKernelGGL((coupling_rqs_dense_h2v2_kernel<A, I, true>), dim3(grid), dim3(FTHREADS), shmem, st, a); \
                              else hipLaunchKernelGGL((coupling_rqs_dense_h2v2_kernel<A, I, false>), dim3(grid), dim3(FTHREADS), shmem, st, a); } while (0)
#else
#define BGK_LAUNCH(A, I) hipLaunchKernelGGL((coupling_rqs_dense_h2v2_kernel<A, I>), dim3(grid), dim3(FTHREADS), shmem, st, a)
#endif
    if (act == 1) { if (inverse) BGK_LAUNCH(1, 1); else BGK_LAUNCH(1, 0); }
    else if (act == 2) { if (inverse) BGK_LAUNCH(2, 1); else BGK_LAUNCH(2, 0); }
    else { if (inverse) BGK_LAUNCH(3, 1); else BGK_LAUNCH(3, 0); }
#undef BGK_LAUNCH
    return bgk_launch_status(what);
}
#endif

#if !BGK_V2_SAVE && !BGK_V2_BF16
#if BGK_V2_AFFTRAIN
int bgk_launch_affine_dense_v2_train(const BgkAffTrainSave* save,
                               const float* cond, int64_t ldc, int32_t d_c, int32_t periodic,
#else
int bgk_launch_affine_dense_v2(const float* cond, int64_t ldc, int32_t d_c, int32_t periodic,
#endif
                               const void* sA0, const void* sA1, const void* sA1b, const void* sA2, float sc0, float sc1, float sc1b, float sc2, int32_t s_act,
                               const void* tA0, const void* tA1, const void* tA1b, const void* tA2, float tc0, float tc1, float tc1b, float tc2, int32_t t_act,
                               const float* log_alpha, int32_t preserve_volume, int32_t is_circular, int32_t inverse,
                               const float* y, int64_t ldy, int64_t B, int32_t d,
                               float* out, int64_t ldo, float* dlogp, int32_t accumulate, void* stream, const BgkCondSegs* segs) {
#if BGK_V2_AFFTRAIN
    const char* what = "bgk_coupling_affine_dense_h2_train";
#else
    const char* what = "bgk_coupling_affine_dense_h2";
#endif
    AffV2Args a;
    const int n_in = periodic ? 2 * d_c : d_c;
    BGK_CHECK_ARG(make_cond_segs(a.cs, cond, ldc, d_c, segs), "%s: bad conditioning segments", what);
    a.d_c = d_c; a.periodic = periodic; a.S0 = (n_in + 1 + 15) / 16;
#if BGK_V2_AFFTRAIN
    a.shift = AffV2Net{(const uint4*)sA0, (const uint4*)sA1, (const uint4*)sA1b, (const uint4*)sA2, sc0, sc1, sc1b, sc2, save->s_cs, save->s_z0, save->s_z1};
    a.scale = AffV2Net{(const uint4*)tA0, (const uint4*)tA1, (const uint4*)tA1b, (const uint4*)tA2, tc0, tc1, tc1b, tc2, save->t_cs, save->t_z0, save->t_z1};
    a.mu_out = save->mu; a.s_out = save->s_raw; a.ldms = save->ldms; a.zt = save->ldz == 64 ? 2 : 4;
#else
    a.shift = AffV2Net{(const uint4*)sA0, (const uint4*)sA1, (const uint4*)sA1b, (const uint4*)sA2, sc0, sc1, sc1b, sc2};
    a.scale = AffV2Net{(const uint4*)tA0, (const uint4*)tA1, (const uint4*)tA1b, (const uint4*)tA2, tc0, tc1, tc1b, tc2};
#endif
    a.has_shift = sA0 != nullptr; a.has_scale = tA0 != nullptr;
    const bool deep = a.has_shift ? sA1b != nullptr : tA1b != nullptr;
#if BGK_V2_AFFTRAIN
    if (deep) return BGK_EUNSUPPORTED;
    BGK_CHECK_ARG((!a.has_shift || (save->s_z0 && save->s_z1 && save->mu)) && (!a.has_scale || (save->t_z0 && save->t_z1 && save->s_raw)),
                  "%s: null save buffer", what);
    BGK_CHECK_ARG(save->ldz == 64 || save->ldz == 128, "%s: ldz = %lld (64 | 128)", what, (long long)save->ldz);
    BGK_CHECK_ARG(save->ldms >= 32 * ((d + 31) / 32) && save->ldms % 4 == 0 && save->ldms < (1 << 20), "%s: ldms = %lld (a multiple of 4, >= 32 ceil(d / 32))",
                  what, (long long)save->ldms);
#endif
    if (a.has_shift && a.has_scale && (sA1b != nullptr) != (tA1b != nullptr)) return BGK_EUNSUPPORTED;
    const int as = a.has_shift ? s_act : t_act, at = a.has_scale ? t_act : s_act;
    if (!((as == at && as >= 1 && as <= 3) || (as == 2 && at == 3))) return BGK_EUNSUPPORTED;
    a.log_alpha = log_alpha; a.preserve_volume = preserve_volume; a.is_circular = is_circular; a.inverse = inverse;
    a.y = y; a.ldy = ldy; a.B = B; a.d = d; a.out = out; a.ldo = ldo; a.dlogp = dlogp; a.accumulate = accumulate;
    a.magic_d = magic_div(d);
    const int OT = (d + 31) / 32;
    TilePlan tp = plan_tiles(a.cs, d_c, periodic, y, ldy, out, ldo, d, 32 * 128);
    a.nfs = tp.nfs; a.ys = tp.ys; a.stage = tp.stage; a.y_dma = tp.y_dma; a.out_lin = tp.out_lin;
    const int tile_f = 32 * a.nfs + (a.stage == 2 ? 32 * d_c : 0) + 16, park_f = d * SROW;
    a.lds_tile = (((tile_f > park_f ? tile_f : park_f) + 3) / 4) * 4;
#if BGK_V2_AFFTRAIN
    a.slab = a.lds_tile;
    a.lds_tile += 16 * 32;
#endif
    a.lds_per_wave = a.lds_tile + ((32 * a.ys + 3) / 4) * 4;
    const size_t shmem = sizeof(float) * (size_t)FW * a.lds_per_wave;
    const int64_t n_wg = ((B + 31) / 32 + FW - 1) / FW;
    BGK_CHECK_ARG(n_wg < (int64_t)0x7fffffff, "%s: batch too large for one launch", what);
    BGK_CHECK_ARG(ldy < (1 << 24) && ldo < (1 << 24) && (int64_t)32 * d_c < 4096 && (int64_t)32 * d < 4096
                  && OT >= 1 && OT <= 3, "%s: outside the kernel's envelope", what);
    if (shmem > 160 * 1024) {
        bgk_set_error("%s: %d input features / %d dims do not fit the LDS tiles", what, n_in, d);
        return BGK_EUNSUPPORTED;
    }
    hipStream_t st = (hipStream_t)stream;
#define BGK_LAUNCH(S, T, O, D) do { if (shmem > 64 * 1024) (void)hipFuncSetAttribute(reinterpret_cast<const void*>(coupling_affine_dense_v2_kernel<S, T, O, D>), \
                                        hipFuncAttributeMaxDynamicSharedMemorySize, 160 * 1024); \
                                    hipLaunchKernelGGL((coupling_affine_dense_v2_kernel<S, T, O, D>), dim3((int)n_wg), dim3(FTHREADS), shmem, st, a); } while (0)
#if BGK_V2_AFFTRAIN
#define BGK_LAUNCH_D(S, T, O) BGK_LAUNCH(S, T, O, false)
#else
#define BGK_LAUNCH_D(S, T, O) do { if (deep) BGK_LAUNCH(S, T, O, true); else BGK_LAUNCH(S, T, O, false); } while (0)
#endif
#define BGK_LAUNCH_O(S, T) do { if (OT == 1) BGK_LAUNCH_D(S, T, 1); else if (OT == 2) BGK_LAUNCH_D(S, T, 2); else BGK_LAUNCH_D(S, T, 3); } while (0)
// ... 8 lines not shown
```

bgflow_amd/csrc/bgk_pack.hip:

```cpp
#include "bgk_common.h"

namespace {

__device__ __forceinline__ uint16_t pk_bf16_rne(float v) {
    const uint32_t u = __builtin_bit_cast(uint32_t, v);
    return (uint16_t)((u + 0x7fffu + ((u >> 16) & 1u)) >> 16);
}
__device__ __forceinline__ float pk_bf16_to_f32(uint16_t h) { return __builtin_bit_cast(float, (uint32_t)h << 16); }
__device__ __forceinline__ uint16_t pk_part(float v, int p, int bf16) {
    if (bf16) {
        const uint16_t h = pk_bf16_rne(v);
        return p ? pk_bf16_rne(v - pk_bf16_to_f32(h)) : h;
    }
    const _Float16 h = (_Float16)v;
    const _Float16 r = p ? (_Float16)(v - (float)h) : h;
    return __builtin_bit_cast(uint16_t, r);
}

struct PackLayer {
    const float* W; const float* b;
    int rows, K;
    const int32_t* row_map;
    int n_groups;
    int NT, S, natural;
// ... 63 lines not shown
            o[e] = pk_part(v * scale, p, L.bf16);
        }
    } else {
        const int m = blk - L.S * L.NT * 2;
#pragma unroll
        for (int e = 0; e < 8; ++e) o[e] = 0;
        if (kb == 0) {
            const int prow = grp * 32 * L.NT + 32 * m + i;
            const int srow = L.row_map ? L.row_map[prow] : (prow < L.rows ? prow : -1);
            if (srow >= 0) {
                const float v = L.b[srow] * scale;
                o[0] = pk_part(v, 0, L.bf16);
                o[1] = pk_part(v, 1, L.bf16);
            }
        }
    }
    _Float16* dst = L.out + ((int64_t)(grp * blocks_per_group + blk) * 64 + lane) * 8;
    *reinterpret_cast<uint4*>(dst) = *reinterpret_cast<const uint4*>(o);
}

__global__ __launch_bounds__(256) void pack_blocks_kernel(PackGroup g, const float* cs) { pack_blocks_body(g, cs, (int)blockIdx.x); }

constexpr int PACK_MANY = 16;
struct PackOne { PackGroup g; float* cs; };
struct PackMany { PackOne c[PACK_MANY]; };
typedef const __attribute__((address_space(4))) PackMany* packmany_t;

__global__ __launch_bounds__(1024) void pack_maxscale_many_kernel(PackMany) {
    const packmany_t ka = (packmany_t)__builtin_amdgcn_kernarg_segment_ptr();
    const int layer = blockIdx.x, ci = blockIdx.y;
    const float* W = ka->c[ci].g.L[layer].W;
    const float* b = ka->c[ci].g.L[layer].b;
    const int rows = ka->c[ci].g.L[layer].rows, nW = rows * ka->c[ci].g.L[layer].K, bf16 = ka->c[ci].g.L[layer].bf16;
    float* cs = ka->c[ci].cs;
    __shared__ float red[16];
    float m = 0.0f;
    for (int i = threadIdx.x; i < nW; i += 1024) m = fmaxf(m, fabsf(W[i]));
    for (int i = threadIdx.x; i < rows; i += 1024) m = fmaxf(m, fabsf(b[i]));
    for (int off = 32; off > 0; off >>= 1) m = fmaxf(m, __shfl_xor(m, off));
    if ((threadIdx.x & 63) == 0) red[threadIdx.x >> 6] = m;
    __syncthreads();
    if (threadIdx.x == 0) {
        for (int w = 1; w < 16; ++w) m = fmaxf(m, red[w]);
        if (!(m < 3.0e38f)) m = 3.4e38f;
        int e = 0;
        if (!bf16 && m > 0.0f && m < 3.0e38f) {
            e = (int)floorf(log2f(32768.0f / m));
            e = e < -16 ? -16 : (e > 24 ? 24 : e);
        }
        cs[2 * layer] = ldexpf(1.0f, e);
        cs[2 * layer + 1] = ldexpf(1.0f, -e);
    }
}

__global__ __launch_bounds__(256) void pack_blocks_many_kernel(PackMany) {
    const PackMany* km = (const PackMany*)__builtin_amdgcn_kernarg_segment_ptr();
    const int ci = blockIdx.y;
    if ((int)blockIdx.x >= km->c[ci].g.first[3]) return;
    pack_blocks_body(km->c[ci].g, km->c[ci].cs, (int)blockIdx.x);
}

int fill_group(PackGroup& g, const PackLayer& L0, const PackLayer& L1, const PackLayer& L2) {
    g.L[0] = L0; g.L[1] = L1; g.L[2] = L2;
    int blocks = 0;
    for (int q = 0; q < 3; ++q) {
        const PackLayer& L = g.L[q];
        const int blocks_per_group = L.S * L.NT * 2 + (L.natural ? 0 : L.NT);
        const int64_t total = (int64_t)L.n_groups * blocks_per_group * 64;
        g.first[q] = blocks;
        blocks += (int)((total + 255) / 256);
    }
    g.first[3] = blocks;
    return blocks;
}

void launch_pack(const PackLayer& L0, const PackLayer& L1, const PackLayer& L2, const float* cs, hipStream_t st) {
    PackGroup g;
    const int blocks = fill_group(g, L0, L1, L2);
    hipLaunchKernelGGL(pack_blocks_kernel, dim3((unsigned)blocks), dim3(256), 0, st, g, cs);
}

}

extern "C" int bgk_pack_dense_h2(const float* W0, const float* b0, int32_t n_in, int32_t H,
                                 const float* W1, const float* b1,
                                 const float* W2, const float* b2, int32_t rows2,
                                 const int32_t* row_map2_dev, int32_t n_groups2, int32_t NT2, int32_t operand_dtype,
                                 void* A0, void* A1, void* A2, float* cs, void* stream) {
    BGK_CHECK_ARG(W0 && b0 && W1 && b1 && W2 && b2 && A0 && A1 && A2 && cs, "bgk_pack_dense_h2: null pointer");
    BGK_CHECK_ARG(n_in > 0 && (H == 32 || H == 64 || H == 96 || H == 128) && rows2 > 0 && n_groups2 > 0 && NT2 > 0 && NT2 <= 4,
                  "bgk_pack_dense_h2: bad sizes");
    hipStream_t st = (hipStream_t)stream;
    const int HT = H / 32;
    BGK_CHECK_ARG(operand_dtype == 0 || operand_dtype == 1, "bgk_pack_dense_h2: operand_dtype %d (0 = split-f16, 1 = bf16)", operand_dtype);
    PackLayer L0{W0, b0, H, n_in, nullptr, 1, HT, (n_in + 1 + 15) / 16, 1, (_Float16*)A0, operand_dtype};
    PackLayer L1{W1, b1, H, H, nullptr, 1, HT, 2 * HT, 0, (_Float16*)A1, operand_dtype};
    PackLayer L2{W2, b2, rows2, H, row_map2_dev, n_groups2, NT2, 2 * HT, 0, (_Float16*)A2, operand_dtype};
    if (hipMemsetAsync(cs, 0, 6 * sizeof(float), st) != hipSuccess) { bgk_set_error("bgk_pack_dense_h2: memset failed"); return BGK_EINVAL; }
    hipLaunchKernelGGL(pack_max_kernel, dim3(3 * PACK_SPLIT), dim3(256), 0, st, L0, L1, L2, cs);
    hipLaunchKernelGGL(pack_scale_kernel, dim3(1), dim3(64), 0, st, L0, L1, L2, cs);
    launch_pack(L0, L1, L2, cs, st);
    return bgk_launch_status("bgk_pack_dense_h2");
}

extern "C" int bgk_pack_mlp_h2(const float* W0, const float* b0, int32_t n_in, int32_t H0,
                               const float* W1, const float* b1, int32_t H1,
                               const float* W2, const float* b2, int32_t rows2,
                               const int32_t* row_map2_dev, int32_t n_groups2, int32_t NT2, int32_t HT,
                               void* A0, void* A1, void* A2, float* cs, void* stream) {
    BGK_CHECK_ARG(W0 && b0 && W1 && b1 && W2 && b2 && A0 && A1 && A2 && cs, "bgk_pack_mlp_h2: null pointer");
    BGK_CHECK_ARG(n_in > 0 && HT >= 1 && HT <= 4 && H0 > 0 && H0 <= 32 * HT && H1 > 0 && H1 <= 32 * HT && rows2 > 0 && n_groups2 > 0
                  && NT2 > 0 && NT2 <= 4, "bgk_pack_mlp_h2: bad sizes");
    hipStream_t st = (hipStream_t)stream;
    PackLayer L0{W0, b0, H0, n_in, nullptr, 1, HT, (n_in + 1 + 15) / 16, 1, (_Float16*)A0, 0};
    PackLayer L1{W1, b1, H1, H0, nullptr, 1, HT, 2 * HT, 0, (_Float16*)A1, 0};
    PackLayer L2{W2, b2, rows2, H1, row_map2_dev, n_groups2, NT2, 2 * HT, 0, (_Float16*)A2, 0};
    if (hipMemsetAsync(cs, 0, 6 * sizeof(float), st) != hipSuccess) { bgk_set_error("bgk_pack_mlp_h2: memset failed"); return BGK_EINVAL; }
    hipLaunchKernelGGL(pack_max_kernel, dim3(3 * PACK_SPLIT), dim3(256), 0, st, L0, L1, L2, cs);
    hipLaunchKernelGGL(pack_scale_kernel, dim3(1), dim3(64), 0, st, L0, L1, L2, cs);
    launch_pack(L0, L1, L2, cs, st);
    return bgk_launch_status("bgk_pack_mlp_h2");
}

extern "C" int bgk_pack_mlp_h2_many(int32_t n, const float* const* W0, const float* const* b0, const int32_t* n_in, const int32_t* H0,
                                    const float* const* W1, const float* const* b1, const int32_t* H1,
                                    const float* const* W2, const float* const* b2,
                                    const int32_t* rows2, const int32_t* const* row_map2_dev, const int32_t* n_groups2, const int32_t* NT2,
                                    const int32_t* HT,
                                    void* const* A0, void* const* A1, void* const* A2, float* const* cs, void* stream) {
    BGK_CHECK_ARG(n >= 0 && W0 && b0 && n_in && W1 && b1 && W2 && b2 && rows2 && row_map2_dev && n_groups2 && A0 && A1 && A2 && cs,
                  "bgk_pack_mlp_h2_many: null pointer");
    if (n == 0) return 0;
    hipStream_t st = (hipStream_t)stream;
    for (int base = 0; base < n; base += PACK_MANY) {
        const int cnt = n - base < PACK_MANY ? n - base : PACK_MANY;
        PackMany M;
        int max_blocks = 0;
        for (int c = 0; c < cnt; ++c) {
            const int i = base + c;
            const int h0 = H0 ? H0[i] : 128, h1 = H1 ? H1[i] : 128, nt2 = NT2 ? NT2[i] : 4, ht = HT ? HT[i] : 4;
            BGK_CHECK_ARG(W0[i] && b0[i] && W1[i] && b1[i] && W2[i] && b2[i] && A0[i] && A1[i] && A2[i] && cs[i] && n_in[i] > 0 && rows2[i] > 0
                          && n_groups2[i] > 0 && ht >= 1 && ht <= 4 && h0 > 0 && h0 <= 32 * ht && h1 > 0 && h1 <= 32 * ht && nt2 >= 1 && nt2 <= 4,
                          "bgk_pack_mlp_h2_many: bad conditioner %d", i);
            PackLayer L0{W0[i], b0[i], h0, n_in[i], nullptr, 1, ht, (n_in[i] + 1 + 15) / 16, 1, (_Float16*)A0[i], 0};
            PackLayer L1{W1[i], b1[i], h1, h0, nullptr, 1, ht, 2 * ht, 0, (_Float16*)A1[i], 0};
            PackLayer L2{W2[i], b2[i], rows2[i], h1, row_map2_dev[i], n_groups2[i], nt2, 2 * ht, 0, (_Float16*)A2[i], 0};
            const int blocks = fill_group(M.c[c].g, L0, L1, L2);
            M.c[c].cs = cs[i];
            max_blocks = blocks > max_blocks ? blocks : max_blocks;
        }
        for (int c = cnt; c < PACK_MANY; ++c) M.c[c] = M.c[0];
        hipLaunchKernelGGL(pack_maxscale_many_kernel, dim3(3, (unsigned)cnt), dim3(1024), 0, st, M);
        hipLaunchKernelGGL(pack_blocks_many_kernel, dim3((unsigned)max_blocks, (unsigned)cnt), dim3(256), 0, st, M);
    }
    return bgk_launch_status("bgk_pack_mlp_h2_many");
}

extern "C" int bgk_pack_dense_h2_many(int32_t n, const float* const* W0, const float* const* b0, const int32_t* n_in,
                                      const float* const* W1, const float* const* b1, const float* const* W2, const float* const* b2,
                                      const int32_t* rows2, const int32_t* const* row_map2_dev, const int32_t* n_groups2,
                                      void* const* A0, void* const* A1, void* const* A2, float* const* cs, void* stream) {
    return bgk_pack_mlp_h2_many(n, W0, b0, n_in, nullptr, W1, b1, nullptr, W2, b2, rows2, row_map2_dev, n_groups2, nullptr, nullptr, A0, A1, A2, cs, stream);
}
```

bgflow_amd/dense.py:

```python
import ctypes
import os
import weakref

import numpy as np
import torch

from . import _lib
from .utils import is_list_or_tuple, param_pitch, param_state_key, row_pitch

__all__ = ["DenseNet", "MeanFreeDenseNet", "WrapPeriodic", "WrapDistances"]


def _matmul_nn(g, w):
    return torch.nn.functional.linear(g, w.t().contiguous())


def _gram_tn(g, h, splits=64):
    B = g.shape[0]
    if B % splits or B // splits < 256:
        return g.t() @ h
    return torch.bmm(g.view(splits, B // splits, -1).transpose(1, 2), h.view(splits, B // splits, -1)).sum(0)


def column_sum(g, nblk=1024):
# ... 603 lines not shown
    if len(parts) > 1 and plan["hidden"] != 128:
        parts = [x.cat()]
    _lib.require_hip(y, *parts)
    y2, ldy = _lib.rowmajor(y)
    B, d = y2.shape
    if out is None:
        out = torch.empty((B, d), dtype=torch.float32, device=y.device)
    if acc is not None:
        dlogp, accumulate = acc.peek()
    if dlogp is None:
        dlogp, accumulate = torch.empty((B,), dtype=torch.float32, device=y.device), False
    ldo = out.stride(0)
    assert out.shape == (B, d) and out.stride(1) == 1 and dlogp.shape == (B,) and dlogp.is_contiguous()
    if plan.get("anydepth"):
        return _fused_affine_anydepth(transformer, plan, parts[0] if len(parts) == 1 else x.cat(), y2, ldy, B, d, out, ldo, dlogp, accumulate,
                                      inverse, acc)
    args = []
    deep = plan["depth"] == 4
    for entry in plan["packed"]:
        if entry is None:
            args += ([None] * 4 + [1.0] * 4 + [0]) if deep else [None, None, None, 1.0, 1.0, 1.0, 0]
        else:
            packed, act = entry
            if packed[0].device != y.device:
                return None
            A0, A1, A2, (c0, c1, c2) = packed[:4]
            if deep:
                args += [_lib.ptr(A0), _lib.ptr(A1), _lib.ptr(packed[4]), _lib.ptr(A2), c0, c1, packed[5], c2, act]
            else:
                args += [_lib.ptr(A0), _lib.ptr(A1), _lib.ptr(A2), c0, c1, c2, act]
    log_alpha = transformer._log_alpha.detach().to(device=y.device, dtype=torch.float32)
    lib = _lib.lib()
    tail = (*args, plan["hidden"], _lib.ptr(log_alpha), int(transformer._preserve_volume), int(transformer._is_circular), int(inverse),
            _lib.ptr(y2), ldy, B, d, _lib.ptr(out), ldo, _lib.ptr(dlogp), int(bool(accumulate)), _lib.stream_ptr(y.device))
    with torch.cuda.device(y.device):
        st = -2
        if len(parts) > 1:
            ptrs, lds, widths, n, keep = _lib.cond_segments(parts)
            st = (lib.bgk_coupling_affine_dense_h3_mc if deep else lib.bgk_coupling_affine_dense_h2_mc)(
                ptrs, lds, widths, n, int(plan["periodic"]), *tail)
            if st == -2:
                parts = [x.cat()]
        if st == -2:
            x2, ldc = _lib.rowmajor(parts[0])
            st = (lib.bgk_coupling_affine_dense_h3 if deep else lib.bgk_coupling_affine_dense_h2)(
                _lib.ptr(x2), ldc, plan["d_c"], int(plan["periodic"]), *tail)
    if st == -2:
        return _reject(transformer, "shape outside the fused affine kernels' envelope: " + _lib.lib().bgk_last_error().decode(errors="replace"))
    _lib.check(st, "bgk_coupling_affine_dense_h3" if deep else "bgk_coupling_affine_dense_h2")
    if acc is not None:
        acc.commit()
        return out, acc
    return out, dlogp[:, None]


def _fused_affine_anydepth(transformer, plan, x, y2, ldy, B, d, out, ldo, dlogp, accumulate, inverse, acc):
    args, keep = [], []
    for entry in plan["packed"]:
        if entry is None:
            args += [None, None, None, 1.0, None, 1.0, 0]
            continue
        (A0, A1, A2, c0, c1s, c2), act = entry
        if A0.device != y2.device:
            return None
        arr = (ctypes.c_float * max(1, len(c1s)))(*c1s)
        keep.append(arr)
        args += [_lib.ptr(A0), _lib.ptr(A1), _lib.ptr(A2), c0, arr, c2, act]
    log_alpha = transformer._log_alpha.detach().to(device=y2.device, dtype=torch.float32)
    x2, ldc = _lib.rowmajor(x)
    with torch.cuda.device(y2.device):
        st = _lib.lib().bgk_coupling_affine_dense_deep(
            _lib.ptr(x2), ldc, plan["d_c"], int(plan["periodic"]), *args, plan["depth"] - 1, plan["hidden"], _lib.ptr(log_alpha),
            int(transformer._preserve_volume), int(transformer._is_circular), int(inverse),
            _lib.ptr(y2), ldy, B, d, _lib.ptr(out), ldo, _lib.ptr(dlogp), int(bool(accumulate)), _lib.stream_ptr(y2.device))
    if st == -2:
        return _reject(transformer, "shape outside the fused affine kernels' envelope: " + _lib.lib().bgk_last_error().decode(errors="replace"))
    _lib.check(st, "bgk_coupling_affine_dense_deep")
    if acc is not None:
        acc.commit()
        return out, acc
    return out, dlogp[:, None]


def pack_dense_for_fused_h2(linears, nc_slot_host, d, n_bins):
    l0, l1, l2 = linears
    W0, b0 = l0.weight.detach().float(), l0.bias.detach().float()
    W1, b1 = l1.weight.detach().float(), l1.bias.detach().float()
    W2, b2 = l2.weight.detach().float(), l2.bias.detach().float()
    n_in = l0.in_features
    S0 = (n_in + 1 + 15) // 16
    e0, e1, e2 = _h2_scale_exp(W0, b0), _h2_scale_exp(W1, b1), _h2_scale_exp(W2, b2)
    W0e = torch.zeros(128, 16 * S0, dtype=torch.float32, device=W0.device)
    W0e[:, :n_in] = W0
    W0e[:, n_in] = b0
    A0 = _pack_h2(W0e * 2.0 ** e0, None, _h2_k_natural(S0))
    A1 = _pack_h2(W1 * 2.0 ** e1, b1 * 2.0 ** e1, _h2_k_hidden())
    ncp = _lib.lib().bgk_pack_rqs_columns(d, n_bins, None, None)
    src = np.empty(ncp, dtype=np.int32)
    slots = np.ascontiguousarray(nc_slot_host, dtype=np.int32)
    _lib.lib().bgk_pack_rqs_columns(d, n_bins, slots.ctypes.data, src.ctypes.data)
    src_t = torch.as_tensor(src.astype(np.int64), device=W2.device)
    W2r = torch.where(src_t[:, None] >= 0, W2[src_t.clamp_min(0)], torch.zeros((), dtype=W2.dtype, device=W2.device)) * 2.0 ** e2
    b2r = torch.where(src_t >= 0, b2[src_t.clamp_min(0)], torch.zeros((), dtype=b2.dtype, device=b2.device)) * 2.0 ** e2
    A2 = torch.cat([_pack_h2(W2r[c * 128:(c + 1) * 128], b2r[c * 128:(c + 1) * 128], _h2_k_hidden())
                    for c in range(ncp // 128)], dim=0).contiguous()
    return A0, A1, A2, (2.0 ** -e0, 2.0 ** -e1, 2.0 ** -e2)


def pack_dense_for_fused_w256(linears, nc_slot_host, d, n_bins):
    l0, l1, l2 = linears
    W0, b0 = l0.weight.detach().float(), l0.bias.detach().float()
    W1, b1 = l1.weight.detach().float(), l1.bias.detach().float()
    W2, b2 = l2.weight.detach().float(), l2.bias.detach().float()
    assert W0.shape[0] == 256 and W1.shape == (256, 256) and W2.shape[1] == 256
    n_in = l0.in_features
    S0 = (n_in + 1 + 15) // 16
    e0, e1, e2 = _h2_scale_exp(W0, b0), _h2_scale_exp(W1, b1), _h2_scale_exp(W2, b2)
    W0e = torch.zeros(256, 16 * S0, dtype=torch.float32, device=W0.device)
    W0e[:, :n_in] = W0
    W0e[:, n_in] = b0
    kh = _h2_k_hidden(8)
    A0 = torch.cat([_pack_h2(W0e[g * 128:(g + 1) * 128] * 2.0 ** e0, None, _h2_k_natural(S0)) for g in range(2)], dim=0).contiguous()
    A1 = torch.cat([_pack_h2(W1[g * 128:(g + 1) * 128] * 2.0 ** e1, b1[g * 128:(g + 1) * 128] * 2.0 ** e1, kh) for g in range(2)],
                   dim=0).contiguous()
    src_t = _src_col_table(d, n_bins, nc_slot_host, W2.device).to(torch.int64)
    W2r = torch.where(src_t[:, None] >= 0, W2[src_t.clamp_min(0)], torch.zeros((), dtype=W2.dtype, device=W2.device)) * 2.0 ** e2
    b2r = torch.where(src_t >= 0, b2[src_t.clamp_min(0)], torch.zeros((), dtype=b2.dtype, device=b2.device)) * 2.0 ** e2
    A2 = torch.cat([_pack_h2(W2r[c * 128:(c + 1) * 128], b2r[c * 128:(c + 1) * 128], kh)
                    for c in range(src_t.numel() // 128)], dim=0).contiguous()
    return A0, A1, A2, (2.0 ** -e0, 2.0 ** -e1, 2.0 ** -e2)


DEEP_MAX_HIDDEN = 8


def pack_dense_for_fused_deep(linears, nc_slot_host, d, n_bins):
    l0, l_out, mids = linears[0], linears[-1], linears[1:-1]
    W0, b0 = l0.weight.detach().float(), l0.bias.detach().float()
    W2, b2 = l_out.weight.detach().float(), l_out.bias.detach().float()
    n_in = l0.in_features
    S0 = (n_in + 1 + 15) // 16
    e0, e2 = _h2_scale_exp(W0, b0), _h2_scale_exp(W2, b2)
    W0e = torch.zeros(128, 16 * S0, dtype=torch.float32, device=W0.device)
    W0e[:, :n_in] = W0
    W0e[:, n_in] = b0
    A0 = _pack_h2(W0e * 2.0 ** e0, None, _h2_k_natural(S0))
    blocks, c1s = [], []
    for lin in mids:
        W, b = lin.weight.detach().float(), lin.bias.detach().float()
        e = _h2_scale_exp(W, b)
        blocks.append(_pack_h2(W * 2.0 ** e, b * 2.0 ** e, _h2_k_hidden()))
        c1s.append(2.0 ** -e)
    A1 = torch.cat(blocks, dim=0).contiguous() if blocks else None
    src_t = _src_col_table(d, n_bins, nc_slot_host, W2.device).to(torch.int64)
    W2r = torch.where(src_t[:, None] >= 0, W2[src_t.clamp_min(0)], torch.zeros((), dtype=W2.dtype, device=W2.device)) * 2.0 ** e2
    b2r = torch.where(src_t >= 0, b2[src_t.clamp_min(0)], torch.zeros((), dtype=b2.dtype, device=b2.device)) * 2.0 ** e2
    A2 = torch.cat([_pack_h2(W2r[c * 128:(c + 1) * 128], b2r[c * 128:(c + 1) * 128], _h2_k_hidden())
                    for c in range(src_t.numel() // 128)], dim=0).contiguous()
    return A0, A1, A2, 2.0 ** -e0, c1s, 2.0 ** -e2


def pack_dense_for_fused_h2_device(linears, src_col_dev, n_chunks, bufs=None, bf16=False):
    l0, l1, l2 = linears
    dev = l0.weight.device
    n_in = l0.in_features
    S0 = (n_in + 1 + 15) // 16
    if bufs is None:
        A0 = torch.empty((S0 * 8, 64, 8), dtype=torch.float16, device=dev)
        A1 = torch.empty((8 * 8 + 4, 64, 8), dtype=torch.float16, device=dev)
        A2 = torch.empty((n_chunks * (8 * 8 + 4), 64, 8), dtype=torch.float16, device=dev)
        cs = torch.empty(6, dtype=torch.float32, device=dev)
    else:
        A0, A1, A2, cs = bufs
    ws = [t.detach().contiguous() for lin in linears for t in (lin.weight, lin.bias)]
    assert all(w.dtype == torch.float32 for w in ws)
    with torch.cuda.device(dev):
        st = _lib.lib().bgk_pack_dense_h2(
            _lib.ptr(ws[0]), _lib.ptr(ws[1]), n_in, 128, _lib.ptr(ws[2]), _lib.ptr(ws[3]), _lib.ptr(ws[4]), _lib.ptr(ws[5]),
            l2.out_features, _lib.ptr(src_col_dev), n_chunks, 4, int(bf16), _lib.ptr(A0), _lib.ptr(A1), _lib.ptr(A2), _lib.ptr(cs),
            _lib.stream_ptr(dev))
    _lib.check(st, "bgk_pack_dense_h2")
    return A0, A1, A2, cs


T_OPERAND_MAX_IN = 96

BATCHED_REPACK = True

_TRAIN_PLANS = weakref.WeakSet()


def _t_operand_bufs(bufs, P, n_in, dev):
    FT, S2 = (n_in + 31) // 32, ((P + 15) // 16 + 3) // 4 * 4
    key = (P, n_in, str(dev))
    if bufs.get("key") != key:
        bufs.clear()
        bufs.update(key=key, T0=torch.empty((8 * FT * 2 + FT, 64, 8), dtype=torch.float16, device=dev),
                    T1=torch.empty((8 * 8 + 4, 64, 8), dtype=torch.float16, device=dev),
                    T2=torch.empty((S2 * 8 + 4, 64, 8), dtype=torch.float16, device=dev))
    return bufs["T0"], bufs["T1"], bufs["T2"]


def repack_training_plans(param_ids=None):
    if not BATCHED_REPACK:
        return 0
    by_dev = {}
    for tr in list(_TRAIN_PLANS):
        cache = getattr(tr, "_fused_cache", None)
        if not cache or not cache.pop("train_used", False) or cache.get("mode") != "f16x2" or "bufs" not in cache or cache.get("padded"):
            continue
        net = tr._params_net
        inner = net.net if type(net) is WrapPeriodic else net
        spec = _fusable_dense(inner)
        if spec is None:
            continue
        (l0, l1, l2), _ = spec
        params = [p for lin in (l0, l1, l2) for p in (lin.weight, lin.bias)]
        if param_ids is not None and not all(id(p) in param_ids for p in params):
            continue
        if not all(p.is_cuda and p.dtype == torch.float32 and p.is_contiguous() for p in params):
            continue
        version = tuple(param_state_key(p) for p in params)
        if cache.get("version") == version:
            continue
        by_dev.setdefault(params[0].device, []).append((cache, l0, l1, l2, params, version))
    done = 0
    for dev, items in by_dev.items():
        n = len(items)
        vps, i32s = (ctypes.c_void_p * n), (ctypes.c_int32 * n)
        col = lambda f: vps(*[f(it) for it in items])
        with torch.cuda.device(dev):
            st = _lib.lib().bgk_pack_dense_h2_many(
                n, col(lambda it: it[4][0].data_ptr()), col(lambda it: it[4][1].data_ptr()), i32s(*[it[1].in_features for it in items]),
                col(lambda it: it[4][2].data_ptr()), col(lambda it: it[4][3].data_ptr()),
                col(lambda it: it[4][4].data_ptr()), col(lambda it: it[4][5].data_ptr()), i32s(*[it[3].out_features for it in items]),
                col(lambda it: it[0]["src_col_dev"].data_ptr()), i32s(*[it[0]["src_col_dev"].numel() // 128 for it in items]),
                col(lambda it: it[0]["bufs"][0].data_ptr()), col(lambda it: it[0]["bufs"][1].data_ptr()),
                col(lambda it: it[0]["bufs"][2].data_ptr()), col(lambda it: it[0]["bufs"][3].data_ptr()), _lib.stream_ptr(dev))
            _lib.check(st, "bgk_pack_dense_h2_many")
            t_items = [it for it in items if it[1].in_features <= T_OPERAND_MAX_IN]
            if t_items:
                m = len(t_items)
                tb = [_t_operand_bufs(it[0].setdefault("tbufs", {}), it[3].out_features, it[1].in_features, dev) for it in t_items]
                tcol = lambda f: (ctypes.c_void_p * m)(*[f(it) for it in t_items])
                st = _lib.lib().bgk_pack_dense_h2_t_many(
                    m, tcol(lambda it: it[4][0].data_ptr()), (ctypes.c_int32 * m)(*[it[1].in_features for it in t_items]),
                    tcol(lambda it: it[4][2].data_ptr()), tcol(lambda it: it[4][4].data_ptr()),
                    (ctypes.c_int32 * m)(*[it[3].out_features for it in t_items]), tcol(lambda it: it[0]["bufs"][3].data_ptr()),
                    (ctypes.c_void_p * m)(*[t[0].data_ptr() for t in tb]), (ctypes.c_void_p * m)(*[t[1].data_ptr() for t in tb]),
                    (ctypes.c_void_p * m)(*[t[2].data_ptr() for t in tb]), _lib.stream_ptr(dev))
                _lib.check(st, "bgk_pack_dense_h2_t_many")
        for cache, l0, _l1, _l2, _params, version in items:
            cache["version"] = version
            if l0.in_features <= T_OPERAND_MAX_IN:
                cache["tbufs"]["t_version"] = (version[0], version[2], version[4])
        done += n
    return done


def _src_col_table(d, n_bins, nc_slot_host, device):
    ncp = _lib.lib().bgk_pack_rqs_columns(d, n_bins, None, None)
    src = np.empty(ncp, dtype=np.int32)
    slots = np.ascontiguousarray(nc_slot_host, dtype=np.int32)
    _lib.lib().bgk_pack_rqs_columns(d, n_bins, slots.ctypes.data, src.ctypes.data)
    return torch.as_tensor(src, device=device)


def _gemm_mode(transformer):
    mode = getattr(transformer, "gemm_mode", None) or GEMM_MODE
    if mode not in ("f32", "f16x2", "bf16"):
        raise ValueError(f"unknown gemm_mode {mode!r} (expected 'f32', 'f16x2' or 'bf16')")
    return mode


def _fused_plan(transformer, y_dim, nc_slot_host):
    mode = _gemm_mode(transformer)
    net = transformer._params_net
    periodic = False
    if type(net) is WrapPeriodic:
        if not (net.left == 0.0 and net.right == 1.0):
            return _reject(transformer, "WrapPeriodic on an interval other than [0, 1]") if _looks_dense(net) else None
        inner = net.net
        periodic = True
    else:
        inner = net
    spec = _fusable_dense(inner)
    if spec is None:
        deep = _fusable_dense_any(inner)
        if deep is not None and len(deep[0]) - 1 <= DEEP_MAX_HIDDEN and mode == "f16x2" \
                and all(lin.out_features <= 128 for lin in deep[0][:-1]):
            return _deep_plan(transformer, net, deep, periodic, y_dim, nc_slot_host)
        if type(inner) is DenseNet:
            return _reject(transformer, "the fused spline kernels take a DenseNet with biases and one of SiLU / ReLU / Tanh: two hidden "
                                        "layers of up to 256 units, or (mode 'f16x2') 1 .. 8 hidden layers of up to 128")
        return None
    (l0, l1, l2), act = spec
    H_max = max(l0.out_features, l1.out_features)
    if H_max > 256:
        return _reject(transformer, f"hidden layers ({l0.out_features}, {l1.out_features}): widths up to 256 are fused")
    if H_max > 128 and mode != "f16x2":
        return _reject(transformer, f"hidden layers ({l0.out_features}, {l1.out_features}) in gemm_mode '{mode}': widths above 128 are "
                                    f"fused in mode 'f16x2' only")
    H_run = 128 if H_max <= 128 else 256
    padded = (l0.out_features, l1.out_features) != (H_run, H_run)
    if y_dim > 64:
        return _reject(transformer, f"{y_dim} transformed dims: at most 64 are fused")
    n_nc = int((nc_slot_host >= 0).sum())
    P = l2.out_features
    n_bins = (P - n_nc) // (3 * y_dim)
    if 3 * n_bins * y_dim + n_nc != P:
        return None
    if n_bins != 8 and not (n_bins in (4, 12, 16, 32) and mode == "f16x2"):
        return _reject(transformer, f"{n_bins} bins in gemm_mode '{mode}': fused for 8 bins, and for 4 / 12 / 16 / 32 bins in mode 'f16x2'"
                                    + ("; more than 64 bins run on device torch ops" if n_bins > 64 else ""))
    d_c = l0.in_features // 2 if periodic else l0.in_features
    if periodic:
        idx = np.arange(d_c)[net.indices] if not isinstance(net.indices, slice) or net.indices != slice(None) else np.arange(d_c)
        if len(idx) != d_c or 2 * d_c != l0.in_features or not np.array_equal(np.asarray(idx), np.arange(d_c)):
            return _reject(transformer, "WrapPeriodic over a subset / permutation of the conditioner inputs")
    params = [p for lin in (l0, l1, l2) for p in (lin.weight, lin.bias)]
    version = tuple(param_state_key(p) for p in params)
    cache = transformer._fused_cache
    dev = l0.weight.device
    stale = cache.get("version") != version
    if cache.get("y_dim") != y_dim or cache.get("mode") != mode or cache.get("device") != dev:
        cache.clear()
        stale = True
    if stale:
        common = dict(version=version, y_dim=y_dim, mode=mode, device=dev, act=act, periodic=periodic, d_c=d_c, n_bins=n_bins,
                      padded=padded, hidden=H_run, circ_mask=int(sum(1 << j for j in range(y_dim) if nc_slot_host[j] < 0)))
        if padded:
            l0, l1, l2 = _pad_hidden((l0, l1, l2), H_run)
        if mode == "bf16" and dev.type != "cuda":
            return None
        if H_run == 256:
            cache.update(common, packed=pack_dense_for_fused_w256((l0, l1, l2), nc_slot_host, y_dim, n_bins), cs=None)
            cache.pop("bufs", None)
        elif mode == "bf16" or (mode == "f16x2" and dev.type == "cuda"):
            if "src_col_dev" not in cache:
                cache["src_col_dev"] = _src_col_table(y_dim, n_bins, nc_slot_host, dev)
            n_chunks = cache["src_col_dev"].numel() // 128
            A0, A1, A2, cs = pack_dense_for_fused_h2_device((l0, l1, l2), cache["src_col_dev"], n_chunks, cache.get("bufs"),
                                                            bf16=(mode == "bf16"))
            cache.update(common, bufs=(A0, A1, A2, cs), packed=(A0, A1, A2, (1.0, 1.0, 1.0)), cs=cs)
        else:
            pack = pack_dense_for_fused if mode == "f32" else pack_dense_for_fused_h2
            cache.update(common, packed=pack((l0, l1, l2), nc_slot_host, y_dim, n_bins), cs=None)
            cache.pop("bufs", None)
    return cache


def _deep_plan(transformer, net, spec, periodic, y_dim, nc_slot_host):
    lins, act = spec
    if y_dim > 64:
        return _reject(transformer, f"{y_dim} transformed dims: at most 64 are fused")
    n_nc = int((nc_slot_host >= 0).sum())
    P = lins[-1].out_features
    n_bins = (P - n_nc) // (3 * y_dim)
    if 3 * n_bins * y_dim + n_nc != P:
        return None
    if n_bins not in (4, 8, 12, 16, 32):
        return _reject(transformer, f"{n_bins} bins: the one-launch kernels take 4 / 8 / 12 / 16 / 32")
    l0 = lins[0]
    d_c = l0.in_features // 2 if periodic else l0.in_features
    if periodic:
        idx = np.arange(d_c)[net.indices] if not isinstance(net.indices, slice) or net.indices != slice(None) else np.arange(d_c)
        if len(idx) != d_c or 2 * d_c != l0.in_features or not np.array_equal(np.asarray(idx), np.arange(d_c)):
            return _reject(transformer, "WrapPeriodic over a subset / permutation of the conditioner inputs")
    version = tuple(param_state_key(p) for lin in lins for p in (lin.weight, lin.bias))
    cache = transformer._fused_cache
    dev = l0.weight.device
    if cache.get("version") != version or cache.get("y_dim") != y_dim or cache.get("mode") != "f16x2" or cache.get("device") != dev \
            or not cache.get("deep"):
        cache.clear()
        padded = any(lin.out_features != 128 for lin in lins[:-1])
        run = _pad_hidden(lins, 128) if padded else lins
        cache.update(version=version, y_dim=y_dim, mode="f16x2", device=dev, act=act, periodic=periodic, d_c=d_c, n_bins=n_bins,
                     padded=padded, hidden=128, deep=len(lins) - 1, cs=None,
                     circ_mask=int(sum(1 << j for j in range(y_dim) if nc_slot_host[j] < 0)),
                     packed=pack_dense_for_fused_deep(run, nc_slot_host, y_dim, n_bins))
    return cache


def fused_spline_coupling(transformer, x, y, nc_slot_host, inverse, oob_counter, want_bin_idx=False, acc=None):
    if x.dim() != 2 or y.dim() != 2 or not x.is_cuda:
        return None
    plan = _fused_plan(transformer, y.shape[-1], nc_slot_host)
    if plan is None or x.shape[-1] != plan["d_c"]:
        return None
    parts = _cond_parts(x)
    if len(parts) > 1 and (plan["mode"] == "f32" or plan["n_bins"] != 8 or plan["hidden"] != 128 or plan.get("deep")):
        parts = [x.cat()]
    _lib.require_hip(y, *parts)
    W0p, W1p, W2p = plan["packed"][:3]
    if W0p.device != y.device:
        return None
    y2, ldy = _lib.rowmajor(y)
    B, d = y2.shape
    out = torch.empty((B, d), dtype=torch.float32, device=y.device)
    if acc is not None:
        dlogp, accumulate = acc.peek()
    else:
        dlogp, accumulate = torch.empty((B,), dtype=torch.float32, device=y.device), False
    bins = torch.empty((B, d), dtype=torch.int32, device=y.device) if want_bin_idx else None
    s = transformer._default_settings
    tail = (plan["hidden"], plan["hidden"], plan["act"], _lib.ptr(y2), ldy, B, d, plan["n_bins"], plan["circ_mask"], int(inverse),
            transformer._left, transformer._right, transformer._bottom, transformer._top,
            s["min_bin_width"], s["min_bin_height"], s["min_derivative"], int(s.get("enable_identity_init", False)),
            _lib.ptr(out), d, _lib.ptr(dlogp), int(bool(accumulate)), _lib.ptr(bins), _lib.ptr(oob_counter), _lib.stream_ptr(y.device))
    with torch.cuda.device(y.device):
        if plan.get("deep"):
            A0, A1, A2, c0, c1s, c2 = plan["packed"]
            x2, ldc = _lib.rowmajor(parts[0])
            c1_arr = (ctypes.c_float * max(1, len(c1s)))(*c1s)
            st = _lib.lib().bgk_coupling_rqs_dense_deep(
                _lib.ptr(x2), ldc, plan["d_c"], int(plan["periodic"]), _lib.ptr(A0), _lib.ptr(A1), _lib.ptr(A2), c0, c1_arr, c2,
                plan["deep"], *tail[2:])
        elif plan["mode"] == "f32":
            x2, ldc = _lib.rowmajor(parts[0])
            st = _lib.lib().bgk_coupling_rqs_dense(
                _lib.ptr(x2), ldc, plan["d_c"], int(plan["periodic"]), _lib.ptr(W0p), _lib.ptr(W1p), _lib.ptr(W2p), *tail)
        else:
            c0, c1, c2 = plan["packed"][3]
            ops = (_lib.ptr(W0p), _lib.ptr(W1p), _lib.ptr(W2p), c0, c1, c2, _lib.ptr(plan.get("cs")), int(plan["mode"] == "bf16"))
            st = -2
            if len(parts) > 1:
                ptrs, lds, widths, n, keep = _lib.cond_segments(parts)
                st = _lib.lib().bgk_coupling_rqs_dense_h2_mc(ptrs, lds, widths, n, int(plan["periodic"]), *ops, *tail)
                if st == -2:
                    parts = [x.cat()]
            if st == -2:
                x2, ldc = _lib.rowmajor(parts[0])
                st = _lib.lib().bgk_coupling_rqs_dense_h2(_lib.ptr(x2), ldc, plan["d_c"], int(plan["periodic"]), *ops, *tail)
    if st == -2:
        return _reject(transformer, "shape outside the fused spline kernels' envelope: " + _lib.lib().bgk_last_error().decode(errors="replace"))
    _lib.check(st, "bgk_coupling_rqs_dense")
    if acc is not None:
        acc.commit()
    res = (out, acc if acc is not None else dlogp[:, None])
    return res + (bins,) if want_bin_idx else res


def _act_fwd_bwd(code):
    if code == 1:
        return torch.nn.functional.silu, lambda g, z, h: torch.ops.aten.silu_backward(g, z)
    if code == 2:
        return torch.relu, lambda g, z, h: g * (z > 0).to(g.dtype)
    return torch.tanh, lambda g, z, h: g * (1.0 - h * h)


def _featurise(x, periodic):
    if not periodic:
        return x
    ang = 2 * np.pi * x
    return torch.cat([torch.cos(ang), torch.sin(ang)], dim=-1)


PACKED_PARAMS = True
RECOMPUTE_PARAMS = True


def absmax_of(*tensors):
    dev = next(t for t in tensors if t is not None).device
    out = torch.zeros(len(tensors), dtype=torch.float32, device=dev)
    with torch.cuda.device(dev):
        for i, t in enumerate(tensors):
            if t is None or t.numel() == 0:
                continue
            t2, ld = _lib.rowmajor(t.detach())
            _lib.check(_lib.lib().bgk_absmax(_lib.ptr(t2), ld, t2.shape[0], t2.shape[1], _lib.ptr(out[i:]), _lib.stream_ptr(dev)), "bgk_absmax")
    return out


def _dense_backward_dx(g_p, z1, z0, x, W0, W1, W2, cs, act_code, periodic, want_gx, bufs, want_h=True, t_version=None, absmax=None,
                       gx_add=None, gx_out=None):
    dev = g_p.device
    B, P = g_p.shape
    n_in = W0.shape[1]
    _t_operand_bufs(bufs, P, n_in, dev)
    T0, T1, T2 = bufs["T0"], bufs["T1"], bufs["T2"]
    g2, ldg = _lib.rowmajor(g_p)
    x2, ldc = _lib.rowmajor(x.detach())
    d_c = x2.shape[1]
    n_out = 4 if want_h else 2
    out = torch.empty((n_out, B, 128), dtype=torch.float32, device=dev)
    g_x = (gx_out if gx_out is not None else torch.empty((B, d_c), dtype=torch.float32, device=dev)) if want_gx else None
    add2, lda = _lib.rowmajor(gx_add) if (gx_add is not None and want_gx) else (None, 0)
    ws = [w.detach().contiguous() for w in (W0, W1, W2)]
    with torch.cuda.device(dev):
        if t_version is None or bufs.get("t_version") != t_version:
            st = _lib.lib().bgk_pack_dense_h2_t(_lib.ptr(ws[0]), n_in, _lib.ptr(ws[1]), _lib.ptr(ws[2]), P, _lib.ptr(cs),
                                                _lib.ptr(T0), _lib.ptr(T1), _lib.ptr(T2), _lib.stream_ptr(dev))
            _lib.check(st, "bgk_pack_dense_h2_t")
            bufs["t_version"] = t_version
        st = _lib.lib().bgk_dense_backward_dx(_lib.ptr(g2), ldg, P, _lib.ptr(z1), _lib.ptr(z0), _lib.ptr(x2), ldc, d_c, int(periodic),
                                              _lib.ptr(T0), _lib.ptr(T1), _lib.ptr(T2), _lib.ptr(cs), act_code, B,
                                              _lib.ptr(out[0]), _lib.ptr(out[1]), _lib.ptr(out[2]) if want_h else None,
                                              _lib.ptr(out[3]) if want_h else None, _lib.ptr(g_x), _lib.rowmajor(g_x)[1] if g_x is not None else d_c,
                                              _lib.ptr(add2), lda, _lib.ptr(absmax), _lib.ptr(absmax[1:]) if absmax is not None else None, _lib.stream_ptr(dev))
        _lib.check(st, "bgk_dense_backward_dx")
    return out[0], out[1], (out[2] if want_h else None), (out[3] if want_h else None), g_x


_DIRECT_GRADS = [False]


DEFERRED_WGRAD_REDUCE = True

_PENDING_REDUCE = {}


def flush_weight_grad_reductions():
    if not _PENDING_REDUCE:
        return
    by_dev = {}
    for dev, *rest in _PENDING_REDUCE.values():
# ... 863 lines not shown
```

include/bgflow_amd.h:

```cpp
#ifndef BGFLOW_AMD_H
#define BGFLOW_AMD_H

#include <stdint.h>

#ifdef __cplusplus
extern "C" {
#endif

#pragma GCC visibility push(default)

#define BGK_EINVAL (-1)
#define BGK_EUNSUPPORTED (-2)

int bgk_abi_version(void);
const char* bgk_last_error(void);

int bgk_set_option(int32_t option, int32_t value);

int bgk_detmath_probe(const float* x, int64_t n, int32_t which, float* out, void* stream);

int bgk_rqs_transform(const float* y, int64_t ldy, const float* params, int64_t ldp, int32_t P,
                      const int32_t* nc_slot, int64_t B, int32_t d, int32_t K, int32_t inverse,
                      double left, double right, double bottom, double top,
                      double min_bin_width, double min_bin_height, double min_derivative,
// ... 312 lines not shown
               uint64_t seed, uint32_t offset, int64_t row0, int64_t B,
               float* dlogp, int32_t accumulate, double logdet, int32_t* bad_count, void* stream);

int64_t bgk_dense_weight_grad_workspace(int64_t B, int32_t P, int32_t n_in);
int bgk_dense_weight_grad(const float* g_params, int64_t ldg, int32_t P, const float* g_z1, const float* g_z0,
                          const float* h1, const float* h0, int32_t h_act, const float* cond, int64_t ldc, int32_t d_c,
                          int32_t periodic, int64_t B, float* workspace, int64_t workspace_floats,
                          float* gW2, float* gb2, float* gW1, float* gb1, float* gW0, float* gb0, int32_t accumulate,
                          const float* g_absmax, void* stream);
int bgk_dense_weight_grad_reduce_many(int32_t n, const int64_t* B, const int32_t* P, const int32_t* n_in,
                                      float* const* workspace, float* const* gW2, float* const* gb2, float* const* gW1,
                                      float* const* gb1, float* const* gW0, float* const* gb0, int32_t accumulate, void* stream);

int64_t bgk_mlp_weight_grad_workspace(int64_t B, int32_t P, int32_t H1, int32_t H0, int32_t n_in);
int bgk_mlp_weight_grad(const float* g_out, int64_t ldg, int32_t P, const float* g_z1, const float* g_z0,
                        const float* h1, const float* h0, int64_t ldz, int32_t H1, int32_t H0, int32_t h_act,
                        const float* cond, int64_t ldc, int32_t d_c, int32_t periodic, int64_t B,
                        float* workspace, int64_t workspace_floats,
                        float* gW2, float* gb2, float* gW1, float* gb1, float* gW0, float* gb0, int32_t accumulate,
                        const float* g_absmax, void* stream);
int bgk_mlp_weight_grad_reduce_many(int32_t n, const int64_t* B, const int32_t* P, const int32_t* H1, const int32_t* H0,
                                    const int32_t* n_in, float* const* workspace, float* const* gW2, float* const* gb2,
                                    float* const* gW1, float* const* gb1, float* const* gW0, float* const* gb0,
                                    int32_t accumulate, void* stream);

int bgk_coupling_affine_dense_fwd64_train(const float* cond, int64_t ldc, int32_t n_in,
                                          const void* sA0, const void* sA1, const void* sA2, const float* s_cs, int32_t s_act,
                                          const void* tA0, const void* tA1, const void* tA2, const float* t_cs, int32_t t_act,
                                          const float* log_alpha, int32_t preserve_volume, int32_t is_circular, int32_t inverse,
                                          const float* y, int64_t ldy, int64_t B, int32_t d, float* out, int64_t ldo,
                                          float* dlogp, int32_t accumulate,
                                          float* s_z0, float* s_z1, float* t_z0, float* t_z1, float* mu, float* s_raw, int64_t ldms,
                                          void* stream);

int64_t bgk_affine_net_backward64_workspace(int64_t B, int32_t d, int32_t H1, int32_t H0, int32_t n_in);
int bgk_affine_net_backward64(const float* g, int64_t ldg, int32_t d, const float* z1, const float* z0,
                              const float* cond, int64_t ldc, int32_t n_in, int32_t H1, int32_t H0,
                              const void* T0, const void* T1, const void* T2, const float* cs, int32_t act, int64_t B,
                              float* g_cond, int64_t ldgc, const float* g_cond_add, int64_t ldga, const float* g_absmax,
                              float* workspace, int64_t workspace_floats,
                              float* gW2, float* gb2, float* gW1, float* gb1, float* gW0, float* gb0, int32_t accumulate,
                              void* stream);

int64_t bgk_affine_coupling_backward64_workspace(int64_t B, int32_t d, int32_t n_in, int32_t sH1, int32_t sH0, int32_t tH1, int32_t tH0);
int bgk_affine_coupling_backward64(const float* cond, int64_t ldc, int32_t n_in, const float* y, int64_t ldy, int32_t d,
                                   const float* g_out, int64_t ldgo, const float* g_dlogp,
                                   const float* s_z0, const float* s_z1, const float* t_z0, const float* t_z1, const float* s_raw, int64_t lds,
                                   const void* sA0, const void* sA1, const void* sT0, const void* sT1, const void* sT2,
                                   const float* s_cs, int32_t s_act, int32_t sH1, int32_t sH0,
                                   const void* tA0, const void* tA1, const void* tA2, const void* tT0, const void* tT1, const void* tT2,
                                   const float* t_cs, int32_t t_act, int32_t tH1, int32_t tH0,
                                   const float* log_alpha, int32_t inverse, int64_t B,
                                   float* g_y, int64_t ldgy, float* g_mu, float* g_cond, int64_t ldgc, const float* g_cond_add, int64_t ldga,
                                   float* g_log_alpha, float* workspace, int64_t workspace_floats,
                                   float* const* s_grads, float* const* t_grads, int32_t accumulate, void* stream);

int64_t bgk_linear_weight_grad_workspace(int64_t B, int32_t n, int32_t k);
int bgk_linear_weight_grad(const float* g, int64_t ldg, int32_t n, const float* h, int64_t ldh, int32_t k, int64_t B,
                           float* workspace, int64_t workspace_floats, float* gW, float* gb, int32_t accumulate,
                           const float* g_absmax, void* stream);

int bgk_column_sum(const float* x, int64_t ldx, int64_t B, int32_t P, float* partial, int32_t nblk,
                   float* out, void* stream);

int bgk_absmax(const float* x, int64_t ldx, int64_t B, int32_t P, float* out, void* stream);

int bgk_dense_layer(const float* x, int64_t ldx, int64_t B, int32_t n_in, const void* Ap, int32_t S, float c, const float* c_dev,
                    const float* bias, int32_t n_out, int32_t act, float* y, int64_t ldy, int32_t accumulate, void* stream);

int bgk_pack_linear_layer(const float* W, int64_t ldw, int32_t n_out, int32_t n_in, void* Ap, float* cs, void* stream);

int bgk_dense_layer_steps(int32_t n_in);
int bgk_refresh_linear_layer(const float* W, int64_t ldw, int32_t n_out, int32_t n_in, int32_t transposed, void* Ap, float* cs, void* state,
                             void* stream);
int bgk_activation(const float* z, int64_t ldz, int64_t B, int32_t n, int32_t act, float* out, int64_t ldo, void* stream);
int bgk_activation_backward(const float* z, int64_t ldz, const float* g, int64_t ldg, int64_t B, int32_t n, int32_t act,
                            float* g_z, int64_t ldgz, void* stream);

int bgk_whiten(const float* x, int64_t ldx, const float* T, const float* pre, const float* post,
               int32_t n_in, int32_t n_out, int64_t B, float* out, int64_t ldo, void* stream);

int32_t bgk_pack_rqs_columns(int32_t d, int32_t K, const int32_t* nc_slot_host, int32_t* src_col);

#pragma GCC visibility pop

#ifdef __cplusplus
}
#endif
#endif
```

Measured before the change: 132.7 million.

## Permute output-layer rows so spline bin params stay in MFMA registers

Adds a second row order for the packed output-layer weights. Under this order the MFMA accumulator tiles hold each dimension's width and height logits directly in registers, so the spline reads them from registers and only slopes and leftovers go through LDS. A new REGP kernel instance uses this order, with a LiveTM pipeline that interleaves loading and computing the next chunk's tiles. The Python side packs a second, permuted weight copy and tries it first, falling back to the old path when it is rejected. This is meant to cut LDS writes and reads per chunk. The cost is an extra packed weight copy and more kernel instances.

```diff
diff --git a/bgflow_amd/_lib.py b/bgflow_amd/_lib.py
--- a/bgflow_amd/_lib.py
+++ b/bgflow_amd/_lib.py
@@ -124,6 +124,7 @@
     "bgk_dense_weight_grad": (ctypes.c_int, [vp, i64, i32, vp, vp, vp, vp, i32, vp, i64, i32, i32, i64, vp, i64,
                                              vp, vp, vp, vp, vp, vp, i32, vp, vp]),
     "bgk_pack_rqs_columns": (i32, [i32, i32, vp, vp]),
+    "bgk_pack_rqs_columns_v": (i32, [i32, i32, vp, i32, vp, vp]),
     "bgk_dense_layer": (ctypes.c_int, [vp, i64, i64, i32, vp, i32, f32, vp, vp, i32, i32, vp, i64, i32, vp]),
     "bgk_pack_linear_layer": (ctypes.c_int, [vp, i64, i32, i32, vp, vp, vp]),
     "bgk_dense_layer_steps": (ctypes.c_int, [i32]),
diff --git a/bgflow_amd/csrc/bgk_fused.hip b/bgflow_amd/csrc/bgk_fused.hip
--- a/bgflow_amd/csrc/bgk_fused.hip
+++ b/bgflow_amd/csrc/bgk_fused.hip
@@ -1309,11 +1309,13 @@
               float* z0, float* z1, float* params, int64_t ldp, const int32_t* src_col, void* stream, const BgkCondSegs* segs = nullptr,
               int params_layout = 0) {
     if (segs && segs->n >= 1) { cond = segs->ptr[0]; ldc = segs->ld[0]; }
+    const int row_order = operand_dtype == 2 ? 2 : 1;
+    if (operand_dtype == 2) operand_dtype = 0;
     BGK_CHECK_ARG(cond && A0p && A1p && A2p && y && out && dlogp, "%s: null pointer", what);
     BGK_CHECK_ARG(B >= 0 && d > 0 && d_c > 0, "%s: bad sizes", what);
     const bool other_k = (K == 4 || K == 12 || K == 16 || K == 32) && operand_dtype == 0;
     const bool wide = H0 == 32 * W_T && H1 == 32 * W_T;
-    if (wide && (operand_dtype != 0 || z0 || z1 || params || (segs && segs->n > 1))) {
+    if (wide && (operand_dtype != 0 || row_order != 1 || z0 || z1 || params || (segs && segs->n > 1))) {
         bgk_set_error("%s: hidden width 256 runs fused in split-f16 inference from one conditioning tensor only", what);
         return BGK_EUNSUPPORTED;
     }
@@ -1364,6 +1366,10 @@
         return bgk_launch_status(what);
     }
     const bool v2_ok = bgk_h2_variant == 2 && K == KB && ldc < (1 << 24) && ldy < (1 << 24) && ldo < (1 << 24);
+    if (row_order == 2 && !(v2_ok && z0 == nullptr)) {
+        bgk_set_error("%s: output-layer row order 2 is read by the second-generation inference kernel only (8 bins, hidden width 128)", what);
+        return BGK_EUNSUPPORTED;
+    }
     if (segs && segs->n > 1 && !v2_ok) return BGK_EUNSUPPORTED;
     if (params_layout == 1 && !(v2_ok && z0 != nullptr && operand_dtype == 0 && params && z1)) return BGK_EUNSUPPORTED;
     if (params_layout == 2 && !(v2_ok && z0 != nullptr && operand_dtype == 0 && z1)) return BGK_EUNSUPPORTED;
@@ -1379,7 +1385,7 @@
     if (v2_ok && z0 == nullptr && operand_dtype == 0)
         return bgk_launch_rqs_dense_h2v2(what, cond, ldc, d_c, periodic, A0p, A1p, A2p, c0, c1, c2, cs_dev, act, y, ldy, B, d, circ_mask,
                                          inverse, left, right, bottom, top, min_bin_width, min_bin_height, min_derivative,
-                                         identity_init, out, ldo, dlogp, accumulate, bin_idx, oob_count, stream, segs);
+                                         identity_init, out, ldo, dlogp, accumulate, bin_idx, oob_count, stream, segs, row_order);
     FusedArgsH2 ah;
     FusedArgs& a = ah.f;
     a.cond = cond; a.ldc = ldc; a.d_c = d_c; a.periodic = periodic;
diff --git a/bgflow_amd/csrc/bgk_fused2.h b/bgflow_amd/csrc/bgk_fused2.h
--- a/bgflow_amd/csrc/bgk_fused2.h
+++ b/bgflow_amd/csrc/bgk_fused2.h
@@ -11,7 +11,7 @@
                               double left, double right, double bottom, double top,
                               double min_bin_width, double min_bin_height, double min_derivative, int32_t identity_init,
                               float* out, int64_t ldo, float* dlogp, int32_t accumulate, int32_t* bin_idx, int32_t* oob_count,
-                              void* stream, const BgkCondSegs* segs = nullptr);
+                              void* stream, const BgkCondSegs* segs = nullptr, int32_t row_order = 1);
 
 int bgk_launch_rqs_dense_h2v2_train(const char* what, float* z0, float* z1, float* params, int64_t ldp, const int32_t* src_col,
                                     const float* cond, int64_t ldc, int32_t d_c, int32_t periodic,
@@ -20,7 +20,7 @@
                                     double left, double right, double bottom, double top,
                                     double min_bin_width, double min_bin_height, double min_derivative, int32_t identity_init,
                                     float* out, int64_t ldo, float* dlogp, int32_t accumulate, int32_t* bin_idx, int32_t* oob_count,
-                                    void* stream, const BgkCondSegs* segs = nullptr);
+                                    void* stream, const BgkCondSegs* segs = nullptr, int32_t row_order = 1);
 
 int bgk_launch_rqs_bwd_recompute(const char* what, const float* z1, const void* A2p, float c2, const float* cs_dev, int32_t act,
                                  const float* y, int64_t ldy, int64_t B, int32_t d, uint64_t circ_mask, int32_t inverse,
@@ -35,7 +35,7 @@
                                    double left, double right, double bottom, double top,
                                    double min_bin_width, double min_bin_height, double min_derivative, int32_t identity_init,
                                    float* out, int64_t ldo, float* dlogp, int32_t accumulate, int32_t* bin_idx, int32_t* oob_count,
-                                   void* stream, const BgkCondSegs* segs = nullptr);
+                                   void* stream, const BgkCondSegs* segs = nullptr, int32_t row_order = 1);
 
 int bgk_launch_affine_dense_v2(const float* cond, int64_t ldc, int32_t d_c, int32_t periodic,
                                const void* sA0, const void* sA1, const void* sA1b, const void* sA2, float sc0, float sc1, float sc1b, float sc2, int32_t s_act,
diff --git a/bgflow_amd/csrc/bgk_fused2.hip b/bgflow_amd/csrc/bgk_fused2.hip
--- a/bgflow_amd/csrc/bgk_fused2.hip
+++ b/bgflow_amd/csrc/bgk_fused2.hip
@@ -80,6 +80,7 @@
     SpC sc;
     int lds_per_wave;
     int nfs, ys, stage, y_dma, out_lin;
+    int p_floats;
 #if BGK_V2_SAVE
     float* z0; float* z1;
     float* params; int64_t ldp;
@@ -187,6 +188,86 @@
 };
 struct NoLive {
     template <int HK, int NH> __device__ __forceinline__ void hook() {}
+};
+
+template <int NT>
+struct LiveTM {
+    static constexpr int LPT = KS + 1;
+    static constexpr int NLS = LPT * NT;
+    static constexpr int EPT = 3 * KS + 1;
+    static constexpr int NEV = EPT * NT;
+    static constexpr int tile_of(int i) { return NT == 4 ? (i == 0 ? 1 : (i == 1 ? 3 : (i == 2 ? 0 : 2))) : (i == 0 ? 1 : 0); }
+    f32x16 (&out)[4];
+    const BFrag& b;
+    const uint4* W;
+    unsigned voff;
+    TFrag (&ring)[RD];
+    __amdgpu_buffer_rsrc_t rs;
+
+    template <int BLK>
+    __device__ __forceinline__ u32x4 blk() {
+        return __builtin_amdgcn_raw_buffer_load_b128(rs, voff + ((BLK * 1024) & 4095), (BLK * 1024) & ~4095, 0);
+    }
+    template <int L>
+    __device__ __forceinline__ void load() {
+        if constexpr (L < NLS) {
+            constexpr int s = L % LPT, m = tile_of(L / LPT);
+            if constexpr (s < KS) {
+                ring[L % RD].hi = blk<(s * 4 + m) * 2>();
+                ring[L % RD].lo = blk<(s * 4 + m) * 2 + 1>();
+            } else {
+                ring[L % RD].hi = blk<KS * 4 * 2 + m>();
+            }
+        }
+    }
+    template <int L0, int L1>
+    __device__ __forceinline__ void loads() {
+        if constexpr (L0 < L1) { load<L0>(); loads<L0 + 1, L1>(); }
+    }
+    __device__ __forceinline__ void start() {
+        __builtin_amdgcn_sched_barrier(0);
+        rs = __builtin_amdgcn_make_buffer_rsrc((void*)W, 0, 0x7fffffff, 0x00020000);
+        loads<0, RD>();
+        __builtin_amdgcn_sched_barrier(0);
+    }
+    template <int E>
+    __device__ __forceinline__ void event() {
+        __builtin_amdgcn_sched_barrier(0);
+        if constexpr (E < NEV) {
+            constexpr int i = E / EPT, e = E % EPT, m = tile_of(i);
+            if constexpr (e < 3 * KS) {
+                constexpr int s = e / 3, p = e % 3, L = i * LPT + s;
+                const TFrag& f = ring[L % RD];
+                const h16x8 a = __builtin_bit_cast(h16x8, p == 0 ? f.lo : f.hi);
+                const h16x8 bb = p == 1 ? b.lo[s] : b.hi[s];
+                if constexpr (s == 0 && p == 0) {
+                    const f32x16 z = {0.f, 0.f, 0.f, 0.f, 0.f, 0.f, 0.f, 0.f, 0.f, 0.f, 0.f, 0.f, 0.f, 0.f, 0.f, 0.f};
+                    out[m] = __builtin_amdgcn_mfma_f32_32x32x16_f16(a, bb, z, 0, 0, 0);
+                } else {
+                    out[m] = __builtin_amdgcn_mfma_f32_32x32x16_f16(a, bb, out[m], 0, 0, 0);
+                }
+                if constexpr (p == 2) load<L + RD>();
+            } else {
+                constexpr int L = i * LPT + KS;
+                const h16x8 one2 = {(_Float16)1.0f, (_Float16)1.0f, 0, 0, 0, 0, 0, 0};
+                out[m] = __builtin_amdgcn_mfma_f32_32x32x16_f16(__builtin_bit_cast(h16x8, ring[L % RD].hi), one2, out[m], 0, 0, 0);
+                load<L + RD>();
+            }
+        }
+        __builtin_amdgcn_sched_barrier(0);
+    }
+    template <int E0, int E1>
+    __device__ __forceinline__ void events() {
+        if constexpr (E0 < E1) {
+            event<E0>();
+            events<E0 + 1, E1>();
+        }
+    }
+    template <int HK, int NH>
+    __device__ __forceinline__ void hook() {
+        constexpr int e0 = (HK * NEV) / NH, e1 = ((HK + 1) * NEV) / NH;
+        if constexpr (e0 < e1) events<e0, e1>();
+    }
 };
 
 template <class G, int BASE, int NH>
@@ -271,15 +352,10 @@
 };
 
 template <int INV, class H>
-__device__ __forceinline__ float rqs_fast(H hk, float x, const float* pa, const float* pb, const float* ps, bool circ,
+__device__ __forceinline__ float rqs_fast(H hk, float x, const float (&va)[KB], const float (&vb)[KB], const float* ps, int pst, bool circ,
                                           const V2Args& a, const SpK& k, float* lad, int* bin, int* oob) {
     const ScSrc<(BGK_V2_KARG == 2 ? INV != 0 : BGK_V2_KARG != 0)> scs(a);
 #define SC scs.get()
-    float va[KB], vb[KB];
-#pragma unroll
-    for (int i = 0; i < KB; ++i) va[i] = pa[i * ST];
-#pragma unroll
-    for (int i = 0; i < KB; ++i) vb[i] = pb[i * ST];
     *oob = (x < SC.left) | (x > SC.right);
     x = __builtin_amdgcn_fmed3f(x, SC.left, SC.right);
     float mA = __builtin_fmaxf(__builtin_fmaxf(va[0], va[1]), va[2]);
@@ -336,7 +412,7 @@
     *bin = idx;
     hk.template at<11>();
     const int j1 = circ ? ((idx + 1) & 7) : (idx + 1);
-    const float s_lo = ps[idx * ST], s_hi = ps[j1 * ST];
+    const float s_lo = ps[idx * pst], s_hi = ps[j1 * pst];
     const float A_i = hi - lo;
     float mB = __builtin_fmaxf(__builtin_fmaxf(vb[0], vb[1]), vb[2]);
     hk.template at<12>();
@@ -468,7 +544,14 @@
     float lad;
     const float x = s_y[j * a.ys + dim];
     Hooks<G, IT * EH, NHK> hk{g};
-    const float o = rqs_fast<INV>(hk, x, INV ? pw : ph, INV ? ph : pw, ps, circ, a, k, &lad, &bin, &oob);
+    const float* pa = INV ? pw : ph;
+    const float* pb = INV ? ph : pw;
+    float va[KB], vb[KB];
+#pragma unroll
+    for (int i = 0; i < KB; ++i) va[i] = pa[i * ST];
+#pragma unroll
+    for (int i = 0; i < KB; ++i) vb[i] = pb[i * ST];
+    const float o = rqs_fast<INV>(hk, x, va, vb, ps, ST, circ, a, k, &lad, &bin, &oob);
     s_y[valid ? j * a.ys + dim : 32 * a.ys + j] = o;
     oob_local += (valid && j < rows) ? oob : 0;
     bins[IT] = bin;
@@ -529,6 +612,68 @@
     spline_slot<INV, 0, 3 * EH>(g, a, k, s_p, s_y, c, DPC, hh, j, rows, run, oob_local, bins);
     spline_slot<INV, 1, 3 * EH>(g, a, k, s_p, s_y, c, DPC, hh, j, rows, run, oob_local, bins);
     spline_slot<INV, 2, 3 * EH>(g, a, k, s_p, s_y, c, DPC, hh, j, rows, run, oob_local, bins);
+}
+
+constexpr int SLAB = 64 * 32;
+constexpr int SLAB_SLOPES = KB + 1;
+constexpr int SLAB_D4 = 5 * SLAB_SLOPES;
+__device__ __forceinline__ void slab_to_lds(const f32x16 (&h)[4], float* s_p, int hh, int j) {
+#pragma unroll
+    for (int mm = 0; mm < 2; ++mm)
+#pragma unroll
+        for (int r = 0; r < 16; ++r) s_p[drow(mm, r, hh) * 32 + j] = h[1 + 2 * mm][r];
+    __builtin_amdgcn_fence(__ATOMIC_ACQ_REL, "wavefront");
+    __builtin_amdgcn_wave_barrier();
+}
+
+template <int INV, int IT, int NHK, class G>
+__device__ __forceinline__ void spline_slot_reg(G& g, const V2Args& a, const SpK& k, const f32x16& t, const float* s_p, float* s_y, int c, int nd,
+                                                int hh, int j, int rows, float& run, int& oob_local, int (&bins)[3]) {
+    const int q = 2 * IT + hh;
+    const bool valid = q < nd;
+    const int qq = valid ? q : 0;
+    const int dim = c * DPC + qq;
+    const float* ps = s_p + (qq * SLAB_SLOPES) * 32 + j;
+    const bool circ = (a.circ_mask >> dim) & 1ull;
+    int bin, oob;
+    float lad;
+    const float x = s_y[j * a.ys + dim];
+    Hooks<G, IT * EH, NHK> hk{g};
+    float va[KB], vb[KB];
+    if constexpr (IT < 2) {
+#pragma unroll
+        for (int i = 0; i < KB; ++i) { va[i] = INV ? t[i] : t[KB + i]; vb[i] = INV ? t[KB + i] : t[i]; }
+    } else {
+        const float* pw = s_p + SLAB_D4 * 32 + j;
+        const float* pa = INV ? pw : pw + KB * 32;
+        const float* pb = INV ? pw + KB * 32 : pw;
+#pragma unroll
+        for (int i = 0; i < KB; ++i) va[i] = pa[i * 32];
+#pragma unroll
+        for (int i = 0; i < KB; ++i) vb[i] = pb[i * 32];
+    }
+    const float o = rqs_fast<INV>(hk, x, va, vb, ps, 32, circ, a, k, &lad, &bin, &oob);
+    s_y[valid ? j * a.ys + dim : 32 * a.ys + j] = o;
+    oob_local += (valid && j < rows) ? oob : 0;
+    bins[IT] = bin;
+    lad = valid ? lad : 0.0f;
+    float l0 = lad, l1 = lad;
+    asm volatile("s_nop 1\n\tv_permlane32_swap_b32 %0, %1" : "+v"(l0), "+v"(l1));
+    run += l0;
+    run += l1;
+}
+
+template <int INV, int NT>
+__device__ __forceinline__ void chunk_piped_reg(const V2Args& a, const SpK& k, float* s_p, float* s_y, int c, int hh, int j, int rows,
+                                                float& run, int& oob_local, int (&bins)[3], f32x16 (&h)[4], const BFrag& bf,
+                                                TFrag (&ring)[RD], unsigned voff) {
+    LiveTM<NT> g{h, bf, a.A2 + (size_t)(c + 1) * GBLK * 64, voff, ring};
+    g.start();
+    slab_to_lds(h, s_p, hh, j);
+    __builtin_amdgcn_sched_barrier(0);
+    spline_slot_reg<INV, 0, 3 * EH>(g, a, k, h[0], s_p, s_y, c, DPC, hh, j, rows, run, oob_local, bins);
+    spline_slot_reg<INV, 1, 3 * EH>(g, a, k, h[2], s_p, s_y, c, DPC, hh, j, rows, run, oob_local, bins);
+    spline_slot_reg<INV, 2, 3 * EH>(g, a, k, h[2], s_p, s_y, c, DPC, hh, j, rows, run, oob_local, bins);
 }
 
 typedef const __attribute__((address_space(1))) void* gvp_t;
@@ -694,14 +839,15 @@
 #endif
 }
 
-template <int ACT, int INV, bool SAVEP = true>
+template <int ACT, int INV, bool SAVEP = true, bool REGP = false>
 __global__ __launch_bounds__(FTHREADS, 2) void coupling_rqs_dense_h2v2_kernel(V2Args a) {
+    static_assert(!REGP || (!BGK_V2_SAVE && !BGK_V2_BF16), "row order 2 belongs to the split-f16 inference instance");
     if (a.cs_dev) { a.c0 = a.cs_dev[1]; a.c1 = a.cs_dev[3]; a.c2 = a.cs_dev[5]; }
     asm volatile("s_setreg_imm32_b32 hwreg(HW_REG_MODE, 23, 1), 1");
     extern __shared__ __attribute__((aligned(16))) float smem[];
-    const int wave = threadIdx.x >> 6;
+    const int wave = REGP ? __builtin_amdgcn_readfirstlane((int)(threadIdx.x >> 6)) : (int)(threadIdx.x >> 6);
     float* s_p = smem + (size_t)wave * a.lds_per_wave;
-    float* s_y = s_p + 128 * ST;
+    float* s_y = s_p + (REGP ? a.p_floats : 128 * ST);
     const int d = a.d;
     const int64_t n_tiles = (a.B + 31) / 32;
     const int64_t tile = (int64_t)blockIdx.x * FW + wave;
@@ -805,6 +951,19 @@
     for (int c = 0; c < a.n_chunks; ++c) {
         int bins[3] = {0, 0, 0};
         const int nd = (d - c * DPC) < DPC ? (d - c * DPC) : DPC;
+        if constexpr (REGP) {
+            if (c + 2 < a.n_chunks || (c + 2 == a.n_chunks && a.last_tiles > 2)) {
+                chunk_piped_reg<INV, 4>(a, k, s_p, s_y, c, hh, j, rows, run, oob_local, bins, h, bf, ring, voff);
+            } else if (c + 2 == a.n_chunks) {
+                chunk_piped_reg<INV, 2>(a, k, s_p, s_y, c, hh, j, rows, run, oob_local, bins, h, bf, ring, voff);
+            } else {
+                NoLive none;
+                slab_to_lds(h, s_p, hh, j);
+                spline_slot_reg<INV, 0, 1>(none, a, k, h[0], s_p, s_y, c, nd, hh, j, rows, run, oob_local, bins);
+                if (nd > 2) spline_slot_reg<INV, 1, 1>(none, a, k, h[2], s_p, s_y, c, nd, hh, j, rows, run, oob_local, bins);
+                if (nd > 4) spline_slot_reg<INV, 2, 1>(none, a, k, h[2], s_p, s_y, c, nd, hh, j, rows, run, oob_local, bins);
+            }
+        } else
         if (c + 2 < a.n_chunks || (c + 2 == a.n_chunks && a.last_tiles > 2)) {
             chunk_piped<INV, 4, SAVEP>(a, k, s_p, s_y, c, hh, j, rows, run, oob_local, bins, h, bf, ring, voff, b0);
         } else if (c + 2 == a.n_chunks) {
@@ -833,13 +992,19 @@
         __builtin_amdgcn_fence(__ATOMIC_ACQ_REL, "wavefront");
         __builtin_amdgcn_wave_barrier();
     }
-    if (hh == 0 && j < rows) {
-        if (a.accumulate) a.dlogp[b0 + j] += run; else a.dlogp[b0 + j] = run;
-    }
-    store_tile32(out_t, ldo32, s_y, ys, d, a.magic_d, rows, lane, a.out_lin);
+    int lane_e = lane;
+    if constexpr (REGP) {
+        int zero = 0;
+        asm volatile("" : "+v"(zero));
+        lane_e = (int)__builtin_amdgcn_mbcnt_hi(~0u, __builtin_amdgcn_mbcnt_lo(~0u, (unsigned)zero));
+    }
+    if ((lane_e >> 5) == 0 && (lane_e & 31) < rows) {
+        if (a.accumulate) a.dlogp[b0 + (lane_e & 31)] += run; else a.dlogp[b0 + (lane_e & 31)] = run;
+    }
+    store_tile32(out_t, ldo32, s_y, ys, d, a.magic_d, rows, lane_e, a.out_lin);
     if (a.oob_count && __builtin_amdgcn_ballot_w64(oob_local != 0)) {
         for (int off = 32; off > 0; off >>= 1) oob_local += __shfl_xor(oob_local, off);
-        if (lane == 0) atomicAdd(a.oob_count, oob_local);
+        if (lane_e == 0) atomicAdd(a.oob_count, oob_local);
     }
     V2_TS(5 + a.n_chunks);
   }
@@ -1460,8 +1625,15 @@
                               double left, double right, double bottom, double top,
                               double min_bin_width, double min_bin_height, double min_derivative, int32_t identity_init,
                               float* out, int64_t ldo, float* dlogp, int32_t accumulate, int32_t* bin_idx, int32_t* oob_count,
-                              void* stream, const BgkCondSegs* segs) {
+                              void* stream, const BgkCondSegs* segs, int32_t row_order) {
     V2Args a;
+#if BGK_V2_SAVE || BGK_V2_BF16
+    BGK_CHECK_ARG(row_order == 1, "%s: output-layer row order %d (this instance takes order 1)", what, row_order);
+    constexpr bool regp = false;
+#else
+    BGK_CHECK_ARG(row_order == 1 || row_order == 2, "%s: output-layer row order %d (1 | 2)", what, row_order);
+    const bool regp = row_order == 2;
+#endif
     const int n_in = periodic ? 2 * d_c : d_c;
     BGK_CHECK_ARG(make_cond_segs(a.cs, cond, ldc, d_c, segs), "%s: bad conditioning segments", what);
     a.d_c = d_c; a.periodic = periodic;
@@ -1482,7 +1654,12 @@
     const TilePlan tp = plan_tiles(a.cs, d_c, periodic, y, ldy, out, ldo, d, 128 * ST);
     a.nfs = tp.nfs; a.ys = tp.ys; a.stage = tp.stage; a.y_dma = tp.y_dma; a.out_lin = tp.out_lin;
     BGK_CHECK_ARG(32 * a.nfs + 16 <= 128 * ST, "%s: %d conditioner input features do not fit the LDS tile", what, n_in);
-    a.lds_per_wave = ((128 * ST + 32 * a.ys + 32 + 3) / 4) * 4;
+    a.p_floats = 128 * ST;
+    if (regp) {
+        const int feat = 32 * a.nfs + (a.stage == 2 ? 32 * d_c : 0) + 16;
+        a.p_floats = ((feat > SLAB ? feat : SLAB) + 3) / 4 * 4;
+    }
+    a.lds_per_wave = ((a.p_floats + 32 * a.ys + 32 + 3) / 4) * 4;
 #if BGK_V2_SAVE
     a.z0 = z0; a.z1 = z1; a.params = params; a.ldp = ldp; a.src_col = src_col;
 #endif
@@ -1496,8 +1673,11 @@
 #if BGK_V2_SAVE
 #define BGK_LAUNCH(A, I) do { if (params) hipLaunchKernelGGL((coupling_rqs_dense_h2v2_kernel<A, I, true>), dim3(grid), dim3(FTHREADS), shmem, st, a); \
                               else hipLaunchKernelGGL((coupling_rqs_dense_h2v2_kernel<A, I, false>), dim3(grid), dim3(FTHREADS), shmem, st, a); } while (0)
-#else
+#elif BGK_V2_BF16
 #define BGK_LAUNCH(A, I) hipLaunchKernelGGL((coupling_rqs_dense_h2v2_kernel<A, I>), dim3(grid), dim3(FTHREADS), shmem, st, a)
+#else
+#define BGK_LAUNCH(A, I) do { if (regp) hipLaunchKernelGGL((coupling_rqs_dense_h2v2_kernel<A, I, true, true>), dim3(grid), dim3(FTHREADS), shmem, st, a); \
+                              else hipLaunchKernelGGL((coupling_rqs_dense_h2v2_kernel<A, I>), dim3(grid), dim3(FTHREADS), shmem, st, a); } while (0)
 #endif
     if (act == 1) { if (inverse) BGK_LAUNCH(1, 1); else BGK_LAUNCH(1, 0); }
     else if (act == 2) { if (inverse) BGK_LAUNCH(2, 1); else BGK_LAUNCH(2, 0); }
diff --git a/bgflow_amd/csrc/bgk_pack.hip b/bgflow_amd/csrc/bgk_pack.hip
--- a/bgflow_amd/csrc/bgk_pack.hip
+++ b/bgflow_amd/csrc/bgk_pack.hip
@@ -169,6 +169,45 @@
 
 }
 
+namespace {
+void rqs_row_perm2(int32_t* perm) {
+    for (int i = 0; i < 128; ++i) perm[i] = -1;
+    for (int q = 0; q < 5; ++q)
+        for (int e = 0; e < 25; ++e) {
+            int m, t;
+            if (q < 4 && e < 16) {
+                m = 2 * (q >> 1);
+                t = (e & 3) + 8 * (e >> 2) + 4 * (q & 1);
+            } else {
+                const int sigma = e >= 16 ? 9 * q + (e - 16) : 45 + e;
+                m = 1 + 2 * (sigma >> 5);
+                t = sigma & 31;
+            }
+            perm[32 * m + t] = 25 * q + e;
+        }
+}
+}
+
+extern "C" int32_t bgk_pack_rqs_columns_v(int32_t d, int32_t K, const int32_t* nc_slot_host, int32_t row_order, int32_t* src_col, int32_t* perm128) {
+    if (row_order == 1) {
+        if (perm128) for (int i = 0; i < 128; ++i) perm128[i] = i;
+        return bgk_pack_rqs_columns(d, K, nc_slot_host, src_col);
+    }
+    if (row_order != 2 || K != 8 || d <= 0) return BGK_EINVAL;
+    int32_t perm[128];
+    rqs_row_perm2(perm);
+    if (perm128) for (int i = 0; i < 128; ++i) perm128[i] = perm[i];
+    const int ncp = bgk_pack_rqs_columns(d, K, nullptr, nullptr);
+    if (src_col) {
+        int32_t* tmp = new int32_t[ncp];
+        bgk_pack_rqs_columns(d, K, nc_slot_host, tmp);
+        for (int c = 0; c < ncp / 128; ++c)
+            for (int i = 0; i < 128; ++i) src_col[c * 128 + i] = perm[i] >= 0 ? tmp[c * 128 + perm[i]] : -1;
+        delete[] tmp;
+    }
+    return ncp;
+}
+
 extern "C" int bgk_pack_dense_h2(const float* W0, const float* b0, int32_t n_in, int32_t H,
                                  const float* W1, const float* b1,
                                  const float* W2, const float* b2, int32_t rows2,
diff --git a/bgflow_amd/dense.py b/bgflow_amd/dense.py
--- a/bgflow_amd/dense.py
+++ b/bgflow_amd/dense.py
@@ -709,7 +709,7 @@
     return out, dlogp[:, None]
 
 
-def pack_dense_for_fused_h2(linears, nc_slot_host, d, n_bins):
+def pack_dense_for_fused_h2(linears, nc_slot_host, d, n_bins, row_order=1):
     l0, l1, l2 = linears
     W0, b0 = l0.weight.detach().float(), l0.bias.detach().float()
     W1, b1 = l1.weight.detach().float(), l1.bias.detach().float()
@@ -722,11 +722,8 @@
     W0e[:, n_in] = b0
     A0 = _pack_h2(W0e * 2.0 ** e0, None, _h2_k_natural(S0))
     A1 = _pack_h2(W1 * 2.0 ** e1, b1 * 2.0 ** e1, _h2_k_hidden())
-    ncp = _lib.lib().bgk_pack_rqs_columns(d, n_bins, None, None)
-    src = np.empty(ncp, dtype=np.int32)
-    slots = np.ascontiguousarray(nc_slot_host, dtype=np.int32)
-    _lib.lib().bgk_pack_rqs_columns(d, n_bins, slots.ctypes.data, src.ctypes.data)
-    src_t = torch.as_tensor(src.astype(np.int64), device=W2.device)
+    src_t = _src_col_table(d, n_bins, nc_slot_host, W2.device, row_order).to(torch.int64)
+    ncp = src_t.numel()
     W2r = torch.where(src_t[:, None] >= 0, W2[src_t.clamp_min(0)], torch.zeros((), dtype=W2.dtype, device=W2.device)) * 2.0 ** e2
     b2r = torch.where(src_t >= 0, b2[src_t.clamp_min(0)], torch.zeros((), dtype=b2.dtype, device=b2.device)) * 2.0 ** e2
     A2 = torch.cat([_pack_h2(W2r[c * 128:(c + 1) * 128], b2r[c * 128:(c + 1) * 128], _h2_k_hidden())
@@ -885,12 +882,34 @@
     return done
 
 
-def _src_col_table(d, n_bins, nc_slot_host, device):
-    ncp = _lib.lib().bgk_pack_rqs_columns(d, n_bins, None, None)
+def _src_col_table(d, n_bins, nc_slot_host, device, row_order=1):
+    ncp = _lib.lib().bgk_pack_rqs_columns_v(d, n_bins, None, row_order, None, None)
+    if ncp <= 0:
+        raise ValueError(f"no row order {row_order} for {n_bins} bins")
     src = np.empty(ncp, dtype=np.int32)
     slots = np.ascontiguousarray(nc_slot_host, dtype=np.int32)
-    _lib.lib().bgk_pack_rqs_columns(d, n_bins, slots.ctypes.data, src.ctypes.data)
+    _lib.lib().bgk_pack_rqs_columns_v(d, n_bins, slots.ctypes.data, row_order, src.ctypes.data, None)
     return torch.as_tensor(src, device=device)
+
+
+def rqs_row_perm(row_order):
+    perm = np.empty(128, dtype=np.int32)
+    if _lib.lib().bgk_pack_rqs_columns_v(1, 8, None, row_order, None, perm.ctypes.data) <= 0:
+        raise ValueError(f"no row order {row_order}")
+    return perm
+
+
+REGISTER_PARAMS = True
+
+
+def _regparam_operands(plan):
+    if plan.get("regp_version") != plan["version"]:
+        if "src_col_dev2" not in plan:
+            plan["src_col_dev2"] = _src_col_table(plan["y_dim"], plan["n_bins"], plan["regp_slots"], plan["device"], 2)
+        plan["regp_bufs"] = pack_dense_for_fused_h2_device(plan["regp_linears"], plan["src_col_dev2"], plan["src_col_dev2"].numel() // 128,
+                                                           plan.get("regp_bufs"))
+        plan["regp_version"] = plan["version"]
+    return plan["regp_bufs"]
 
 
 def _gemm_mode(transformer):
@@ -970,6 +989,8 @@
             A0, A1, A2, cs = pack_dense_for_fused_h2_device((l0, l1, l2), cache["src_col_dev"], n_chunks, cache.get("bufs"),
                                                             bf16=(mode == "bf16"))
             cache.update(common, bufs=(A0, A1, A2, cs), packed=(A0, A1, A2, (1.0, 1.0, 1.0)), cs=cs)
+            if mode == "f16x2" and n_bins == 8:
+                cache.update(regp_linears=(l0, l1, l2), regp_slots=np.array(nc_slot_host, dtype=np.int32))
         else:
             pack = pack_dense_for_fused if mode == "f32" else pack_dense_for_fused_h2
             cache.update(common, packed=pack((l0, l1, l2), nc_slot_host, y_dim, n_bins), cs=None)
@@ -1050,15 +1071,20 @@
         else:
             c0, c1, c2 = plan["packed"][3]
             ops = (_lib.ptr(W0p), _lib.ptr(W1p), _lib.ptr(W2p), c0, c1, c2, _lib.ptr(plan.get("cs")), int(plan["mode"] == "bf16"))
+            ops_try = [ops]
+            if REGISTER_PARAMS and "regp_linears" in plan and plan["hidden"] == 128:
+                R0, R1, R2, rcs = _regparam_operands(plan)
+                ops_try.insert(0, (_lib.ptr(R0), _lib.ptr(R1), _lib.ptr(R2), c0, c1, c2, _lib.ptr(rcs), 2))
             st = -2
-            if len(parts) > 1:
-                ptrs, lds, widths, n, keep = _lib.cond_segments(parts)
-                st = _lib.lib().bgk_coupling_rqs_dense_h2_mc(ptrs, lds, widths, n, int(plan["periodic"]), *ops, *tail)
+            for ops in ops_try:
+                if len(parts) > 1:
+                    ptrs, lds, widths, n, keep = _lib.cond_segments(parts)
+                    st = _lib.lib().bgk_coupling_rqs_dense_h2_mc(ptrs, lds, widths, n, int(plan["periodic"]), *ops, *tail)
                 if st == -2:
-                    parts = [x.cat()]
-            if st == -2:
-                x2, ldc = _lib.rowmajor(parts[0])
-                st = _lib.lib().bgk_coupling_rqs_dense_h2(_lib.ptr(x2), ldc, plan["d_c"], int(plan["periodic"]), *ops, *tail)
+                    x2, ldc = _lib.rowmajor(x.cat() if len(parts) > 1 else parts[0])
+                    st = _lib.lib().bgk_coupling_rqs_dense_h2(_lib.ptr(x2), ldc, plan["d_c"], int(plan["periodic"]), *ops, *tail)
+                if st != -2:
+                    break
     if st == -2:
         return _reject(transformer, "shape outside the fused spline kernels' envelope: " + _lib.lib().bgk_last_error().decode(errors="replace"))
     _lib.check(st, "bgk_coupling_rqs_dense")
diff --git a/include/bgflow_amd.h b/include/bgflow_amd.h
--- a/include/bgflow_amd.h
+++ b/include/bgflow_amd.h
@@ -418,6 +418,8 @@
 
 int32_t bgk_pack_rqs_columns(int32_t d, int32_t K, const int32_t* nc_slot_host, int32_t* src_col);
 
+int32_t bgk_pack_rqs_columns_v(int32_t d, int32_t K, const int32_t* nc_slot_host, int32_t row_order, int32_t* src_col, int32_t* perm128);
+
 #pragma GCC visibility pop
 
 #ifdef __cplusplus
```

After: 135.2 million, median of 6. 1.02x the previous value.
